# megvii-research/basedet

Hardware: AMD Instinct MI355X
Metric: images/sec training RetinaNet-R50-FPN 1333x800 (higher is better)
Workload: dtype bf16; 1 GPU; retinanet_r50_800x1344 train step (fwd+bwd+allreduce+SGD), DummyLoader boxes, random-init weights, inputs resident in HBM; per_gpu_batch=16, global_batch=16, parallelism=dp1

## Files before the change

basedet_amd/_lib.py:

```python
import ctypes as C
import os

import torch

_HERE = os.path.dirname(os.path.abspath(__file__))
LIB_PATH = os.environ.get("BASEDET_HIP_LIB") or os.path.join(_HERE, "lib", "libbasedet_hip.so")

BD_MAX_SEGS = 8
ABI_VERSION = 105
EPI_RELU, EPI_ADD_BEFORE, EPI_ADD_AFTER, EPI_MASK, EPI_SPARSE = 1, 2, 4, 8, 16


class BasedetHipError(RuntimeError):
    pass


class ConvDesc(C.Structure):
    _fields_ = [
        ("N", C.c_int32), ("Cin", C.c_int32), ("Cout", C.c_int32), ("R", C.c_int32), ("S", C.c_int32),
        ("stride", C.c_int32), ("pad", C.c_int32), ("nseg", C.c_int32),
        ("Hi", C.c_int32 * BD_MAX_SEGS), ("Wi", C.c_int32 * BD_MAX_SEGS),
        ("Ho", C.c_int32 * BD_MAX_SEGS), ("Wo", C.c_int32 * BD_MAX_SEGS),
        ("in_off", C.c_int32 * BD_MAX_SEGS), ("out_off", C.c_int32 * BD_MAX_SEGS),
        ("in_pix_per_img", C.c_int32), ("out_pix_per_img", C.c_int32),
        ("route", C.c_int32 * 4), ("sr_seed", C.c_uint32),
        ("gskip", C.c_int32), ("gskip_ws", C.c_void_p), ("gskip_ws_bytes", C.c_size_t),
        ("gskip_gmap", C.c_void_p), ("gskip_gmap_bytes", C.c_size_t), ("gskip_dxmap", C.c_void_p), ("gskip_dxmap_bytes", C.c_size_t),
        ("gskip_dx_clean", C.c_int32),
    ]


class PackDesc(C.Structure):
    _fields_ = [("w", C.c_void_p), ("row_scale", C.c_void_p), ("w_fwd", C.c_void_p), ("w_dgrad", C.c_void_p),
                ("Cout", C.c_int32), ("RS", C.c_int32), ("Cin", C.c_int32), ("block_start", C.c_int32)]


class ImageDesc(C.Structure):
    _fields_ = [("offset", C.c_int64), ("src_h", C.c_int32), ("src_w", C.c_int32), ("dst_h", C.c_int32), ("dst_w", C.c_int32),
                ("flip", C.c_int32), ("reserved_", C.c_int32 * 1)]


_P, _I, _L, _F, _Z = C.c_void_p, C.c_int, C.c_int64, C.c_float, C.c_size_t
_D = C.POINTER(ConvDesc)

SIGNATURES = {
    "bd_last_error_string": (C.c_char_p, []),
    "bd_version": (_I, []),
    "bd_conv_last_kernel": (C.c_char_p, []),
    "bd_probe_mfma_rate": (_I, [C.c_double, C.POINTER(C.c_double), C.POINTER(C.c_double), _P]),
    "bd_probe_kernel_clock": (_I, [C.c_char_p, _I, C.POINTER(C.c_double), C.POINTER(C.c_double)]),
    "bd_conv2d_fwd": (_I, [_D, _P, _P, _P, _P, _P, _I, _P]),
    "bd_conv2d_dgrad": (_I, [_D, _P, _P, _P, _P, _P, _I, _P]),
    "bd_conv2d_dgrad_gskip_bytes": (_Z, [_D]),
    "bd_conv2d_gskip_map_bytes": (_Z, [_D, _I]),
    "bd_gskip_map_scan": (_I, [_D, _I, _P, _P, _Z, _P]),
    "bd_conv2d_fwd_bits": (_I, [_D, _P, _P, _P, _P, _P, _P, _I, _P]),
    "bd_conv2d_fwd_ex": (_I, [_D, _P, _P, _P, _P, _P, _P, _P, _F, _I, _P]),
    "bd_conv2d_dgrad_ex": (_I, [_D, _P, _P, _P, _P, _P, _P, _P, _F, _I, _P]),
    "bd_conv2d_dgrad_bits": (_I, [_D, _P, _P, _P, _P, _P, _I, _P]),
    "bd_conv2d_wgrad_workspace_bytes": (_Z, [_D]),
    "bd_conv2d_wgrad": (_I, [_D, _P, _P, _P, _P, _I, _P, _Z, _P]),
    "bd_conv2d_wgrad_bias_workspace_bytes": (_Z, [_D]),
    "bd_conv2d_wgrad_bias": (_I, [_D, _P, _P, _P, _P, _P, _I, _P, _Z, _P]),
    "bd_fpn_deconv_pack": (_I, [_P, _I, _P, _P, _P]),
    "bd_fpn_deconv_fwd": (_I, [_P, _P, _P, _P, _I, _I, _I, _I, _I, _I, _P]),
    "bd_fpn_deconv_dgrad": (_I, [_P, _P, _P, _P, _I, _I, _I, _I, _I, _I, _P]),
    "bd_fpn_deconv_wgrad_workspace_bytes": (_Z, [_I, _I, _I, _I]),
    "bd_fpn_deconv_wgrad": (_I, [_P, _P, _P, _I, _P, _Z, _I, _I, _I, _I, _I, _I, _P]),
    "bd_wgrad_queue_create": (_I, [_P]),
    "bd_wgrad_queue_destroy": (_I, [_P]),
    "bd_wgrad_queue_pending": (_I, [_P]),
    "bd_conv2d_wgrad_queued": (_I, [_P, _D, _P, _P, _P, _P, _P, _I, _P, _Z, _P]),
    "bd_wgrad_queue_flush": (_I, [_P, _P]),
    "bd_stem_conv7x7_fwd": (_I, [_I, _I, _I, _P, _P, _P, _P, _P]),
    "bd_stem_pool_fwd": (_I, [_I, _I, _I, _P, _P, _P, _P, _P]),
    "bd_stem_weight_pack": (_I, [_P, _P, _P, _P]),
    "bd_weight_pack": (_I, [_P, _P, _P, _P, _I, _I, _I, _P]),
    "bd_weight_pack_blocks": (_I, [_I, _I, _I]),
    "bd_weight_pack_multi": (_I, [_P, _I, _I, _P]),
    "bd_colsum_workspace_bytes": (_Z, [_I]),
    "bd_colsum_bf16": (_I, [_P, _I, _L, _L, _L, _I, _P, _I, _P, _Z, _P]),
    "bd_pad_normalize": (_I, [_P, _I, _I, _I, _I, _I, _P, _P, _P, _P]),
    "bd_bottleneck_fwd_supported": (_I, [_I, _I, _I, _I, _I, _I, _I]),
    "bd_bottleneck_fwd": (_I, [_I, _I, _I, _I, _I, _I, _P, _P, _P, _P, _P, _P, _P, _P, _P, _P, _P]),
    "bd_h2d_create": (_I, [C.POINTER(C.c_void_p), _I, _I]),
    "bd_h2d_threads": (_I, [_P]),
    "bd_h2d_submit": (_I, [_P, _P, _I, _L, _P, _L, _P]),
    "bd_h2d_destroy": (_I, [_P]),
    "bd_pad_normalize_nchw": (_I, [_P, _I, _I, _I, _I, _I, _P, _P, _P, _P]),
    "bd_resize_pad_normalize": (_I, [_P, _L, C.POINTER(ImageDesc), _I, _I, _I, _P, _P, _P, _P]),
    "bd_maxpool3x3s2_fwd": (_I, [_P, _I, _I, _I, _I, _P, _P]),
    "bd_upsample2x_add_fwd": (_I, [_P, _L, _L, _P, _L, _L, _I, _I, _I, _I, _P]),
    "bd_upsample2x_add_bwd": (_I, [_P, _L, _L, _P, _L, _L, _I, _I, _I, _I, _I, _P]),
    "bd_relu_bf16": (_I, [_P, _P, _L, _P]),
    "bd_relu_bwd_bf16": (_I, [_P, _P, _P, _P, _L, _P]),
    "bd_add_bf16": (_I, [_P, _P, _P, _L, _P]),
    "bd_anchors_generate": (_I, [_I, _I, _I, _F, _P, _I, _P, _P]),
    "bd_points_generate": (_I, [_I, _I, _I, _F, _I, _P, _P]),
    "bd_box_pairwise": (_I, [_P, _I, _P, _I, _I, _P, _P]),
    "bd_box_encode": (_I, [_P, _P, _L, _P, _P, _P, _P]),
    "bd_box_decode": (_I, [_P, _P, _L, _P, _P, _P, _P]),
    "bd_retina_assign_encode": (_I, [_P, _I, _P, _P, _I, _I, _F, _F, _I, _P, _P, _P, _P, _P, _P, _P, _Z, _P]),
    "bd_fcos_assign": (_I, [_P, _I, _P, _P, _P, _I, _F, _P, _P, _I, _I, _P, _P, _P, _P, _P]),
    "bd_ota_assign_workspace_bytes": (_Z, [_I, _I]),
    "bd_ota_assign": (_I, [_P, _I, _P, _P, _I, _P, _I, _P, _P, _P, _I, _I, _F, _F, _F, _F, _I, _P, _P, _P, _P, _P, _Z, _P]),
    "bd_ota_assign_ld": (_I, [_P, _I, _P, _P, _I, _P, _I, _I, _P, _P, _P, _I, _I, _F, _F, _F, _F, _I, _P, _P, _P, _P, _P, _Z, _P]),
    "bd_ota_sinkhorn_workspace_bytes": (_Z, [_I, _I, _I]),
    "bd_ota_assign_sinkhorn": (_I, [_P, _I, _P, _P, _I, _P, _I, _P, _P, _P, _I, _I, _F, _F, _F, _F, _I, _F, _I, _P, _P, _P, _P, _P, _Z, _P]),
    "bd_ota_assign_sinkhorn_ld": (_I, [_P, _I, _P, _P, _I, _P, _I, _I, _P, _P, _P, _I, _I, _F, _F, _F, _F, _I, _F, _I, _P, _P, _P, _P, _P, _Z, _P]),
    "bd_freeanchor_workspace_bytes": (_Z, [_I, _I, _I, _I]),
    "bd_freeanchor_loss_fwd_bwd": (_I, [_P, _P, _I, _I, _P, _I, _I, _P, _P, _I, _I, _P, _P, _F, _I, _F, _F, _F, _F, _P, _P, _P, _P, _Z, _P]),
    "bd_freeanchor_loss_fwd_bwd_ld": (_I, [_P, _I, _P, _I, _I, _P, _I, _I, _P, _P, _I, _I, _P, _P, _F, _I, _F, _F, _F, _F, _P, _P, _P, _P, _Z, _P]),
    "bd_atss_assign_workspace_bytes": (_Z, [_I, _I]),
    "bd_atss_assign": (_I, [_P, _I, _P, _P, _I, _I, _F, _P, _P, _I, _I, _P, _P, _P, _P, _P, _Z, _P]),
    "bd_nms_workspace_bytes": (_Z, [_I]),
    "bd_batched_nms": (_I, [_P, _P, _P, _I, _F, _I, _P, _P, _P, _Z, _P]),
    "bd_focal_loss_fwd_bwd": (_I, [_P, _P, _L, _I, _F, _F, _P, _I, _F, _P, _P, _P]),
    "bd_focal_loss_fwd_bwd_general": (_I, [_P, _P, _L, _I, _F, _F, _P, _I, _F, _P, _P, _P]),
    "bd_focal_loss_fwd_bwd_ld": (_I, [_P, _P, _L, _I, _I, _F, _F, _P, _I, _F, _P, _P, _I, _P]),
    "bd_smooth_l1_fwd_bwd": (_I, [_P, _P, _P, _L, _I, _I, _F, _P, _I, _F, _P, _P, _P]),
    "bd_loss_grid_cap": (_I, []),
    "bd_iou_ltrb_fwd_bwd": (_I, [_P, _P, _P, _P, _L, _I, _P, _F, _P, _P, _P]),
    "bd_giou_ltrb_fwd_bwd": (_I, [_P, _P, _P, _P, _L, _P, _F, _P, _P, _P]),
    "bd_bce_logits_fwd_bwd": (_I, [_P, _I, _I, _P, _P, _L, _P, _P, _P, _P]),
    "bd_groupnorm_workspace_bytes": (_Z, [_I, _I, _I, _L]),
    "bd_groupnorm_fwd": (_I, [_P, _P, _P, _I, _I, _P, _P, _L, _I, _F, _I, _P, _P, _P, _Z, _P]),
    "bd_conv2d_fwd_gnstats_bytes": (_Z, [_D]),
    "bd_conv2d_fwd_gnstats": (_I, [_D, _P, _P, _P, _P, _P, _Z, _P]),
    "bd_groupnorm_fwd_parts": (_I, [_D, _P, _P, _P, _P, _F, _I, _P, _P, _P]),
    "bd_groupnorm_bwd": (_I, [_P, _P, _P, _P, _P, _I, _I, _P, _P, _L, _I, _I, _P, _P, _P, _I, _P, _Z, _P]),
    "bd_fcos_offsets_fwd": (_I, [_P, _I, _P, _I, _I, _P, _P, _P, _L, _P, _P]),
    "bd_fcos_offsets_workspace_bytes": (_Z, []),
    "bd_fcos_offsets_bwd": (_I, [_P, _I, _P, _I, _I, _P, _P, _P, _L, _P, _P, _P, _P, _P, _Z, _P]),
    "bd_rpn_assign_encode": (_I, [_P, _I, _P, _P, _I, _I, _F, _F, _I, _P, _P, _P, _P, _P, _P, _P, _Z, _P]),
    "bd_sample_labels": (_I, [_P, _P, _P, _I, _I, _I, _I, _P, _P]),
    "bd_segment_topk": (_I, [_P, _I, _I, _L, _I, _I, _I, _I, _P, _P, _I, _F, _I, _P, _P, _P, _P]),
    "bd_nms_batched_workspace_bytes": (_Z, [_I, _I]),
    "bd_nms_batched": (_I, [_P, _P, _P, _I, _I, _F, _I, _I, _P, _P, _P, _Z, _P]),
    "bd_rpn_proposals_workspace_bytes": (_Z, [_I, _I, _P, _I, _I, _I]),
    "bd_rpn_proposals": (_I, [_P, _I, _I, _I, _I, _I, _L, _I, _P, _P, _P, _P, _I, _P, _P, _I, _F, _I, _P, _P, _P, _Z, _P]),
    "bd_rpn_proposals_joint": (_I, [_P, _I, _I, _I, _I, _I, _L, _I, _P, _P, _P, _P, _I, _P, _P, _I, _F, _I, _P, _P, _P, _Z, _P]),
    "bd_rcnn_sample_targets": (_I, [_P, _P, _I, _P, _P, _I, _I, _P, _P, _I, _I, _I, _F, _F, _F, _P, _P, _P, _P, _P, _P, _P, _P]),
    "bd_roi_align_fwd": (_I, [_P, _L, _I, _I, _P, _P, _P, _P, _P, _P, _I, _I, _I, _I, _I, _P, _P]),
    "bd_conv1x1_thin_bwd_workspace_bytes": (_Z, []),
    "bd_conv1x1_thin_fwd": (_I, [_P, _P, _P, _L, _I, _I, _P, _P]),
    "bd_conv1x1_thin_bwd": (_I, [_P, _P, _P, _L, _I, _I, _P, _P, _P, _I, _P, _Z, _P]),
    "bd_roi_align_bwd": (_I, [_P, _L, _I, _I, _P, _P, _P, _P, _P, _P, _I, _I, _I, _I, _I, _P, _P]),
    "bd_roi_align_bwd_bf16_workspace_bytes": (_Z, [_I, _I, _P, _P, _I]),
    "bd_roi_align_bwd_bf16": (_I, [_P, _L, _I, _I, _I, _P, _P, _P, _P, _P, _P, _I, _I, _I, _I, _I, _P, _I, _P, _Z, _P]),
    "bd_subsample2x_fwd": (_I, [_P, _L, _L, _I, _I, _P, _L, _L, _I, _I, _P]),
    "bd_subsample2x_bwd_add": (_I, [_P, _L, _L, _P, _L, _L, _I, _I, _I, _I, _P]),
    "bd_f32_to_bf16": (_I, [_P, _P, _L, _P]),
    "bd_f32_to_bf16_add": (_I, [_P, _P, _L, _P]),
    "bd_rpn_loss_fwd_bwd": (_I, [_P, _I, _I, _I, _I, _P, _P, _L, _F, _P, _P, _P, _P]),
    "bd_rcnn_loss_fwd_bwd": (_I, [_P, _I, _I, _I, _P, _P, _I, _F, _P, _P, _P, _P]),
    "bd_det_scores": (_I, [_P, _P, _I, _I, _L, _I, _P, _P]),
    "bd_det_scores_ld": (_I, [_P, _I, _P, _I, _I, _L, _I, _P, _P]),
    "bd_det_select_workspace_bytes": (_Z, [_I, _I, _L, _I, _I]),
    "bd_det_select": (_I, [_P, _P, _I, _I, _I, _L, _I, _I, _P, _P, _I, _F, _P, _P, _P, _P, _Z, _P]),
    "bd_det_select_ld": (_I, [_P, _I, _P, _I, _I, _I, _L, _I, _I, _P, _P, _I, _F, _P, _P, _P, _P, _Z, _P]),
    "bd_rcnn_predict": (_I, [_P, _I, _I, _I, _P, _P, _I, _I, _P, _P, _P, _P, _P]),
    "bd_det_candidates": (_I, [_I, _P, _P, _P, _I, _I, _P, _I, _P, _P, _I, _I, _P, _P, _P, _P, _P, _P, _P]),
    "bd_det_finalize": (_I, [_P, _P, _P, _P, _P, _I, _P, _P, _P, _P, _P]),
    "bd_det_candidates_batched": (_I, [_I, _P, _P, _P, _I, _I, _I, _P, _I, _P, _P, _L, _I, _I, _P, _P, _P, _L, _P, _P, _P, _P]),
    "bd_det_finalize_batched": (_I, [_P, _P, _P, _P, _P, _I, _I, _I, _P, _I, _P, _P, _P, _P]),
    "bd_sgd_momentum_step": (_I, [_P, _P, _P, _L, _F, _F, _F, _F, _P]),
    "bd_ema_update": (_I, [_P, _P, _L, _F, _F, _P]),
    "bd_sgd_momentum_ema_step": (_I, [_P, _P, _P, _P, _L, _F, _F, _F, _F, _F, _F, _P]),
    "bd_swap_f32": (_I, [_P, _P, _L, _P]),
    "bd_clip_grad_value": (_I, [_P, _L, _F, _F, _F, _P]),
    "bd_clip_grad_norm_workspace_bytes": (_Z, []),
    "bd_clip_grad_norm": (_I, [_P, _L, _F, _F, _F, _P, _P, _Z, _P]),
    "bd_quantize_fp8": (_I, [_P, _L, _F, _P, _P]),
    "bd_weight_pack_fp8": (_I, [_P, _P, _I, _I, _I, _F, _P, _P, _P]),
    "bd_conv2d_fwd_fp8": (_I, [_D, _P, _P, _P, _P, _P, _P, _I, _P]),
    "bd_conv2d_fwd_fp8_ex": (_I, [_D, _P, _P, _P, _P, _P, _P, _P, _F, _I, _P]),
    "bd_quantize_bf8": (_I, [_P, _L, _F, _P, C.c_uint32, _P]),
    "bd_absmax_bf16": (_I, [_P, _L, _P, _P]),
    "bd_weight_pack_fp8_t": (_I, [_P, _P, _I, _I, _I, _F, _P, _P, _P]),
    "bd_conv2d_dgrad_fp8": (_I, [_D, _P, _P, _P, _P, _P, _P, _P, _F, _I, _P]),
    "bd_conv2d_wgrad_fp8_workspace_bytes": (_Z, [_D]),
    "bd_conv2d_wgrad_fp8": (_I, [_D, _P, _P, _F, _P, _P, _I, _P, _Z, _P]),
    "bd_conv1x1_fp8": (_I, [_D, _I, _P, _P, _P, _P, _P, _P, _P, _P, _P, _P, _F, _I, _P]),
    "bd_sigmoid_focal_loss_elem": (_I, [_P, _P, _L, _F, _F, _P, _P, _P, _P]),
    "bd_bce_elem": (_I, [_P, _P, _L, _I, _P, _P, _P, _P]),
    "bd_smooth_l1_elem": (_I, [_P, _P, _L, _F, _P, _P, _P, _P]),
    "bd_iou_loss_ltrb": (_I, [_P, _P, _L, _I, _F, _P, _P, _P, _P, _P]),
    "bd_iou_to_loss": (_I, [_P, _L, _I, _F, _P, _P]),
    "bd_matcher_matrix": (_I, [_P, _I, _L, _P, _P, _I, _I, _P, _P, _P, _P]),
    "bd_assign_roi_levels": (_I, [_P, _I, _I, _I, _I, _P, _P]),
    "bd_roi_pool_max_fwd": (_I, [_P, _I, _I, _I, _I, _P, _I, _F, _I, _I, _P, _P]),
    "bd_comm_unique_id": (_I, [_P]),
    "bd_comm_init": (_I, [C.POINTER(C.c_void_p), _P, _I, _I, _I]),
    "bd_comm_rank": (_I, [_P]),
    "bd_comm_world": (_I, [_P]),
    "bd_comm_stream": (_P, [_P]),
    "bd_comm_bcast": (_I, [_P, _P, _Z, _I, _I, _P]),
    "bd_comm_allreduce": (_I, [_P, _P, _Z, _I, _I, _P]),
    "bd_comm_allreduce_async": (_I, [_P, _P, _Z, _I, _I, C.POINTER(C.c_void_p), _I]),
    "bd_comm_allreduce_async_bf16": (_I, [_P, _P, _P, _Z, _I, C.POINTER(C.c_void_p), _I]),
    "bd_comm_wait": (_I, [_P, _P]),
    "bd_comm_destroy": (_I, [_P]),
}

_lib = None


def load():
# ... 51 lines not shown
```

basedet_amd/csrc/conv3x3_pp.hip:

```cpp
#include "conv3x3_pp128_body.h"

namespace {

constexpr int PH = 4, PW = 16, IH = PH + 2, IW = PW + 2;
constexpr int NPATCH = 4;
constexpr int XROWS = NPATCH * IH * IW;
constexpr int X_PITCH = 144;
constexpr int X_BYTES = XROWS * X_PITCH;
constexpr int XPASSES = 7;
constexpr int TILE_CO = 256;
constexpr int W_SLOT = TILE_CO * 128;
constexpr int NSLOT = 3;
constexpr int W_BYTES = NSLOT * W_SLOT;
constexpr int GTAB_TILES = 16;
constexpr int GTAB_BYTES = GTAB_TILES * NPATCH * 32;
constexpr int LDS_BYTES = W_BYTES + X_BYTES + TILE_CO * 4 + GTAB_BYTES;
constexpr int MAX_SEG = BD_MAX_SEGS;
constexpr int TAIL_CO = 64;

struct PSeg { int patch_start, H, W, pw, src_off, dst_off; float inv_pw; };

struct PParams {
    const bf16_raw* src;
    const bf16_raw* w;
    const float* bias;
    const bf16_raw* add;
    const bf16_raw* mask;
    bf16_raw* dst;
    int CK, CO, flags, nseg;
    int src_ppi, dst_ppi;
    unsigned src_bytes;
    int patches_per_img, total_patches, n_tiles;
    int main_grid;
    int px_tiles;
    int tail_end;
    float inv_ppi;
    PSeg seg[MAX_SEG];
    float* gn_part;
    const int* sp_live;
    const int* sp_list;
    const int* sp_count;
    int sp_keep_dead;
    const int* sp_hdr;
    int* sp_ohdr;
    const int* sp_olist;
    int sp_stride, sp_clean;
};

typedef __attribute__((address_space(3))) void lds_void_t;
typedef __attribute__((address_space(1))) const void glb_void_t;

__device__ __forceinline__ int pp_div(int n, int d, float inv) {
    int q = (int)((float)n * inv);
    const int r = n - q * d;
    q += (r >= d) - (r < 0);
    return q;
}

__device__ __forceinline__ int swz(int row, int chunk) { return row * 128 + ((chunk ^ (row & 7)) << 4); }
__device__ __forceinline__ int colperm(int f) { return f < 4 ? 2 * f : (f < 12 ? 2 * (f - 4) + 1 : 2 * (f - 8)); }
__device__ __forceinline__ int xpos(int chunk) { return (chunk >> 2) * 64 + ((((chunk & 1) << 1) | ((chunk >> 1) & 1)) << 4); }

#ifdef BD_PP_STAMP
__device__ unsigned long long g_pp_stamp[64];
__device__ unsigned long long g_pp_span[2048];
#endif
#ifndef BD_PP_ABLATE
#define BD_PP_ABLATE 0
#endif
__device__ unsigned long long g_pp_clk[2];
#define PP_FENCE() __builtin_amdgcn_sched_barrier(0)
#define PP_BARRIER() do { asm volatile("" ::: "memory"); __builtin_amdgcn_s_barrier(); asm volatile("" ::: "memory"); } while (0)

template <int MODE, bool GNS = false, bool SPARSE = false>
__global__ __launch_bounds__(512, 1) void conv3x3_pp_kernel(const PParams p) {
    extern __shared__ __attribute__((aligned(16))) unsigned char smem[];
    if (!SPARSE && (int)blockIdx.x >= p.main_grid) {
        pp128::body<MODE, TAIL_CO>(p, smem, (int)blockIdx.x - p.main_grid, (int)gridDim.x - p.main_grid, p.total_patches, p.tail_end,
                                   (p.CO + TAIL_CO - 1) / TAIL_CO);
        return;
    }
    if (!SPARSE && blockIdx.x == 0 && threadIdx.x == 0) bd_clk_mark(g_pp_clk, false);
    unsigned char* wbuf = smem;
    unsigned char* xbuf = smem + W_BYTES;
    float* sbias = reinterpret_cast<float*>(smem + W_BYTES + X_BYTES);

#ifdef BD_PP_STAMP
    int st_n = 0;
    const bool st_on = blockIdx.x == 100 % gridDim.x && threadIdx.x == 0;
#define PP_STAMP() do { if (st_on && st_n < 62) g_pp_stamp[st_n] = __builtin_amdgcn_s_memtime(); ++st_n; } while (0)
    PP_STAMP();
    if (st_on) g_pp_stamp[62] = __builtin_amdgcn_s_memrealtime();
    if (threadIdx.x == 0 && blockIdx.x < 1024) g_pp_span[2 * blockIdx.x] = __builtin_amdgcn_s_memrealtime();
#else
#define PP_STAMP() do { } while (0)
#endif
    const int tid = threadIdx.x, lane = tid & 63, wave = __builtin_amdgcn_readfirstlane(tid >> 6);
    const int wm = wave >> 2, wp = wave & 3;
    int bid = blockIdx.x;
    {
        const int nwg = p.main_grid;
        const int q = nwg >> 3, r = nwg & 7, xcd = bid & 7;
        bid = (xcd < r ? xcd * (q + 1) : r * (q + 1) + (xcd - r) * q) + (bid >> 3);
    }
    const int ct = bid % p.n_tiles;
    int pt = bid / p.n_tiles;
    const int pt_step = p.main_grid / p.n_tiles;
    const int co0 = ct * TILE_CO;

    auto zero_dead = [&](int z0, int zn) {
        if (p.sp_keep_dead) return;
        const int cpp = p.CO >> 3;
        const int items = PH * PW * cpp;
        int zt = p.total_patches;
        const int* plist = nullptr;
        if (p.sp_clean) {
            const int oc = __builtin_amdgcn_readfirstlane(p.sp_ohdr[0]) & 1;
            const int pc = __builtin_amdgcn_readfirstlane(p.sp_ohdr[2 + oc]);
            zt = pc < 0 ? 0 : (pc < zt ? pc : zt);
            plist = p.sp_olist + oc * p.sp_stride;
        }
        for (int k0 = 0; z0 + k0 * zn < zt; k0 += 512) {
            const int k = k0 + wave * 64 + lane;
            const int idx = z0 + k * zn;
            int q = idx;
            if (plist) q = idx < zt ? plist[idx] : -1;
            const bool dead = idx < zt && q >= 0 && q < p.total_patches && p.sp_live[q] == 0;
            unsigned long long m = __ballot(dead);
            while (m) {
                const int l = __builtin_ctzll(m);
                m &= m - 1;
                const int qq = __builtin_amdgcn_readfirstlane(__shfl(q, l, 64));
                const int n = qq / p.patches_per_img, rem = qq - n * p.patches_per_img;
                int sgi = 0;
#pragma unroll
                for (int z = 1; z < MAX_SEG; ++z)
                    if (z < p.nseg && rem >= p.seg[z].patch_start) sgi = z;
                const int H = p.seg[sgi].H, W = p.seg[sgi].W, pwn = p.seg[sgi].pw;
                const int local = rem - p.seg[sgi].patch_start, by = local / pwn, bx = local - by * pwn;
                const long long img = (long long)n * p.dst_ppi + p.seg[sgi].dst_off;
                for (int i = lane; i < items; i += 64) {
                    const int px = i / cpp, ch = i - px * cpp;
                    const int y = by * PH + px / PW, x = bx * PW + (px & (PW - 1));
                    if (y < H && x < W)
                        *reinterpret_cast<u32x4_t*>(p.dst + (img + (long long)y * W + x) * p.CO + ch * 8) = (u32x4_t){0u, 0u, 0u, 0u};
                }
            }
        }
    };
    int n_px = p.px_tiles, n_live = p.total_patches;
    int z_first = 0;
    const int* sp_list = p.sp_list;
    if constexpr (SPARSE) {
        if (p.sp_ohdr && blockIdx.x == 0 && threadIdx.x == 0) p.sp_ohdr[1] = 0;
        const int cur = p.sp_hdr ? __builtin_amdgcn_readfirstlane(p.sp_hdr[0]) & 1 : 0;
        const int* cntp = p.sp_hdr ? p.sp_hdr + 2 + cur : p.sp_count;
        n_live = __builtin_amdgcn_readfirstlane(*cntp);
        sp_list += cur * p.sp_stride;
        n_live = __builtin_amdgcn_readfirstlane(n_live < 0 ? 0 : (n_live < p.total_patches ? n_live : p.total_patches));
        n_px = (n_live + NPATCH - 1) / NPATCH;
        z_first = n_px * p.n_tiles < p.main_grid ? n_px * p.n_tiles : p.main_grid;
        if (pt >= n_px) {
            zero_dead(bid - z_first, p.main_grid - z_first);
            return;
        }
    }

    constexpr unsigned X_NONE = 0x80000000u;
    const int x_lds0 = (tid >> 3) * X_PITCH + xpos(tid & 7);
    unsigned x_off[XPASSES];

    int* gtab = reinterpret_cast<int*>(smem + W_BYTES + X_BYTES + TILE_CO * 4);
    const int pt_first = pt;
    auto build_table = [&](int k0) {
        const int k = k0 + (lane >> 2);
        const int ptile = pt_first + k * pt_step;
        int pid = ptile * NPATCH + (lane & (NPATCH - 1));
        if (SPARSE) pid = (ptile < n_px && pid < n_live) ? sp_list[pid] : p.total_patches;
        int vH = 0, vW = 0, vy = 0, vx = 0, vs = 0, vd = 0;
        if (ptile < n_px && pid < p.total_patches) {
            const int n = pp_div(pid, p.patches_per_img, p.inv_ppi);
            const int rem = pid - n * p.patches_per_img;
            int g_start = p.seg[0].patch_start, g_H = p.seg[0].H, g_W = p.seg[0].W, g_pw = p.seg[0].pw;
            int g_src = p.seg[0].src_off, g_dst = p.seg[0].dst_off;
            float g_inv = p.seg[0].inv_pw;
#pragma unroll
            for (int q = 1; q < MAX_SEG; ++q) {
                const bool in = q < p.nseg && rem >= p.seg[q].patch_start;
                g_start = in ? p.seg[q].patch_start : g_start; g_H = in ? p.seg[q].H : g_H; g_W = in ? p.seg[q].W : g_W;
                g_pw = in ? p.seg[q].pw : g_pw; g_src = in ? p.seg[q].src_off : g_src; g_dst = in ? p.seg[q].dst_off : g_dst;
                g_inv = in ? p.seg[q].inv_pw : g_inv;
            }
            const int local = rem - g_start;
            const int by = pp_div(local, g_pw, g_inv), bx = local - by * g_pw;
            vy = by * PH; vx = bx * PW; vH = g_H; vW = g_W;
            vs = n * p.src_ppi + g_src;
            vd = n * p.dst_ppi + g_dst;
        }
        typedef __attribute__((ext_vector_type(4))) int i32x4_t;
        i32x4_t* e = reinterpret_cast<i32x4_t*>(gtab + ((k & (GTAB_TILES - 1)) * NPATCH + (lane & (NPATCH - 1))) * 8);
        e[0] = (i32x4_t){vy, vx, vH, vW};
        e[1] = (i32x4_t){vs, vd, 0, 0};
    };
    auto decode = [&](int k, int& e_oy0, int& e_px0, int& e_H, int& e_W, int& e_dst) {
        int py0[NPATCH], px0[NPATCH], pH[NPATCH], pWd[NPATCH];
        int psrc[NPATCH], pdst[NPATCH];
        int tq = tid;
        asm volatile("" : "+v"(tq));
        {
            typedef __attribute__((ext_vector_type(4))) int i32x4_t;
            const i32x4_t* e = reinterpret_cast<const i32x4_t*>(gtab + ((k & (GTAB_TILES - 1)) * NPATCH + (tq & (NPATCH - 1))) * 8);
            const i32x4_t e0 = e[0], e1 = e[1];
#pragma unroll
            for (int q = 0; q < NPATCH; ++q) {
                py0[q] = __builtin_amdgcn_readlane(e0[0], q); px0[q] = __builtin_amdgcn_readlane(e0[1], q);
                pH[q] = __builtin_amdgcn_readlane(e0[2], q); pWd[q] = __builtin_amdgcn_readlane(e0[3], q);
                psrc[q] = __builtin_amdgcn_readlane(e1[0], q); pdst[q] = __builtin_amdgcn_readlane(e1[1], q);
            }
        }
#pragma unroll
        for (int k = 0; k < XPASSES; ++k) {
            const int row = (tq >> 3) + 64 * k;
            unsigned off = X_NONE;
            if (row < XROWS) {
                const int lo = (64 * k) / (IH * IW), hi = (64 * k + 63) / (IH * IW) < NPATCH ? (64 * k + 63) / (IH * IW) : NPATCH - 1;
                const bool up = row >= hi * (IH * IW);
                const int pk = up ? hi : lo;
                const int rr = row - pk * (IH * IW);
                const int iy = rr / IW, ix = rr - iy * IW;
                const int qy = up ? py0[hi] : py0[lo], qx = up ? px0[hi] : px0[lo], H = up ? pH[hi] : pH[lo];
                const int W = up ? pWd[hi] : pWd[lo], qs = up ? psrc[hi] : psrc[lo];
                const int y = qy - 1 + iy, x = qx - 1 + ix;
                if (y >= 0 && x >= 0 && y < H && x < W) off = (unsigned)((qs + y * W + x) * p.CK + (tq & 7) * 8) * 2u;
            }
            x_off[k] = off;
        }
        e_oy0 = py0[0]; e_px0 = px0[0]; e_H = pH[0]; e_W = pWd[0]; e_dst = pdst[0];
#pragma unroll
        for (int q = 1; q < NPATCH; ++q)
            if (wp == q) { e_oy0 = py0[q]; e_px0 = px0[q]; e_H = pH[q]; e_W = pWd[q]; e_dst = pdst[q]; }
    };
    int c_oy0, c_px0, c_H, c_W, c_dst;
    int kt = 0;
    if (wave == 0) build_table(0);
    asm volatile("s_waitcnt lgkmcnt(0)" ::: "memory");
    PP_BARRIER();
    decode(0, c_oy0, c_px0, c_H, c_W, c_dst);
    const __amdgpu_buffer_rsrc_t x_rsrc =
        __builtin_amdgcn_make_buffer_rsrc(const_cast<bf16_raw*>(p.src), 0, p.src_bytes, 0x00020000);
    u32x4_t rx[XPASSES];
    auto load_x = [&](int cb) {
        int so = cb * 128;
        asm volatile("" : "+s"(so));
        const bool dead = cb * 64 + (tid & 7) * 8 >= p.CK;
#pragma unroll
        for (int k = 0; k < XPASSES; ++k) rx[k] = __builtin_amdgcn_raw_buffer_load_b128(x_rsrc, dead ? X_NONE : x_off[k], so, 0);
    };
    auto write_x = [&]() {
#pragma unroll
        for (int k = 0; k < XPASSES; ++k)
            if (k < XPASSES - 1 || (tid >> 3) + 64 * k < XROWS)
                *reinterpret_cast<u32x4_t*>(xbuf + x_lds0 + k * (64 * X_PITCH)) = rx[k];
    };

    unsigned dma_src[4];
#pragma unroll
    for (int k = 0; k < 4; ++k) {
        const int pc = wave + 8 * k;
        const int lrow = 8 * pc + (lane >> 3);
        const int chunk = (lane & 7) ^ (lane >> 3);
        const int rho = lrow & 15;
        int co = co0 + (lrow & 192) + 32 * ((lrow >> 5) & 1) + 8 * (rho >> 2) + 4 * ((lrow >> 4) & 1) + (rho & 3);
        if (co >= p.CO) co = p.CO - 1;
        dma_src[k] = (unsigned)(co * 9 * p.CK + chunk * 8) * 2u;
    }
    const __amdgpu_buffer_rsrc_t w_rsrc =
        __builtin_amdgcn_make_buffer_rsrc(const_cast<bf16_raw*>(p.w), 0, (unsigned)(p.CO * 9 * p.CK) * 2u, 0x00020000);
    bool dma_on = true;
    auto dma_piece = [&](int tap, int cb, int slot, int k) {
        if ((BD_PP_ABLATE & 2) && !dma_on) return;
        unsigned char* l = wbuf + slot * W_SLOT + (wave + 8 * k) * 1024;
        int so = (tap * p.CK + cb * 64) * 2;
        asm volatile("" : "+s"(so));
        __builtin_amdgcn_raw_ptr_buffer_load_lds(w_rsrc, (lds_void_t*)l, 16, dma_src[k], so, 0, 0);
    };

    f32x4_t acc[8][4];

    const int frow = lane & 15, fchunk = lane >> 4;
    const unsigned char* a_base[2];
#pragma unroll
    for (int kk = 0; kk < 2; ++kk) a_base[kk] = wbuf + swz(wm * 128 + frow, kk * 4 + fchunk);
    typedef __attribute__((address_space(3))) const unsigned char lds_u8_t;
    typedef __attribute__((address_space(3))) const bf16x8_t lds_bf16x8_t;
    unsigned a_hi[2];
#pragma unroll
    for (int kk = 0; kk < 2; ++kk) {
        a_hi[kk] = (unsigned)(size_t)(lds_u8_t*)(a_base[kk]) + 2 * W_SLOT;
        asm volatile("" : "+v"(a_hi[kk]));
    }
    const unsigned char* b_base = xbuf + (wp * (IH * IW) + colperm(frow)) * X_PITCH + xpos(fchunk);

    bf16x8_t fa[8], fb[4];
    auto load_a = [&](int kk, int slot) {
#pragma unroll
        for (int i = 0; i < 8; ++i) {
            if (slot == 2) fa[i] = *(lds_bf16x8_t*)(size_t)(a_hi[kk] + i * 2048);
// ... 271 lines not shown
                if (add_before) {
#pragma unroll
                    for (int k = 0; k < 4; ++k) { v[2 * k] += bf_lo(a4[k]); v[2 * k + 1] += bf_hi(a4[k]); }
                }
                if (do_relu) {
#pragma unroll
                    for (int k = 0; k < 8; ++k) v[k] = fmaxf(v[k], 0.f);
                }
                if (do_mask) {
#pragma unroll
                    for (int k = 0; k < 4; ++k) {
                        if (!(bf_lo(m4[k]) > 0.f)) v[2 * k] = 0.f;
                        if (!(bf_hi(m4[k]) > 0.f)) v[2 * k + 1] = 0.f;
                    }
                }
                if (add_after) {
#pragma unroll
                    for (int k = 0; k < 4; ++k) { v[2 * k] += bf_lo(a4[k]); v[2 * k + 1] += bf_hi(a4[k]); }
                }
                u32x4_t o;
#pragma unroll
                for (int k = 0; k < 4; ++k) o[k] = pack_bf2(v[2 * k], v[2 * k + 1]);
                *reinterpret_cast<u32x4_t*>(p.dst + idx) = o;
            }
        }
    }
    }
    PP_STAMP();
    if (!more) break;
    ++kt;
    pt = pt_next;
    c_oy0 = n_oy0; c_px0 = n_px0; c_H = n_H; c_W = n_W; c_dst = n_dst;
    PP_FENCE();
    PP_STAMP();
    }
    if constexpr (SPARSE) {
        if (z_first == p.main_grid) zero_dead(bid, p.main_grid);
    }
    if (!SPARSE && blockIdx.x == 0 && threadIdx.x == 0) bd_clk_mark(g_pp_clk, true);
#ifdef BD_PP_STAMP
    if (st_on) { g_pp_stamp[63] = __builtin_amdgcn_s_memrealtime(); g_pp_stamp[61] = __builtin_amdgcn_s_memtime(); }
    if (threadIdx.x == 0 && blockIdx.x < 1024) { asm volatile("s_waitcnt vmcnt(0)" ::: "memory"); g_pp_span[2 * blockIdx.x + 1] = __builtin_amdgcn_s_memrealtime(); }
#endif
}

}

BD_KNOB int g_pp_tail_split = 1;
BD_KNOB int g_pp_persistent = 1;
extern BD_KNOB int g_patch_pp;
int bd_gskip_patches(const bd_conv_desc* d, int ph, int pw);
void bd_gskip_fill(const bd_conv_desc* d, int side, const void* t, const int* live_in, int* map, hipStream_t stream);
void bd_gskip_scan(const bd_conv_desc* d, const void* g, int ph, int pw, int* mask, hipStream_t stream);
void bd_gskip_compact(const bd_conv_desc* d, int ph, int pw, const int* mask, int* live, int* list, int* count, hipStream_t stream);

extern "C" size_t bd_conv2d_dgrad_gskip_bytes(const bd_conv_desc* d) {
    if (!d || d->nseg < 1 || d->nseg > BD_MAX_SEGS || !(d->R == 3 && d->S == 3 && d->stride == 1 && d->pad == 1)) return 0;
    return ((size_t)3 * bd_gskip_patches(d, PH, PW) + 4) * sizeof(int);
}

static bool pp_sparse_epilogue(int flags, const void* add, const void* dst) {
    const bool in_place = (flags & BD_EPI_ADD_BEFORE) && add && add == dst;
    return !(flags & BD_EPI_ADD_AFTER) && (!((flags & BD_EPI_ADD_BEFORE) && add) || (in_place && !(flags & BD_EPI_MASK)));
}

bool bd_conv3x3_pp_maps_ok(const bd_conv_desc* d, int flags, const void* add, const void* dst) {
    if (g_patch_pp < 2 || !(d->R == 3 && d->S == 3 && d->stride == 1 && d->pad == 1)) return false;
    if (d->Cout % 8 != 0 || d->Cin <= 128 || d->Cin % 8 != 0) return false;
    if ((long long)d->N * d->out_pix_per_img * d->Cout * 2 >= 0x7fffffffll || (long long)d->N * d->in_pix_per_img >= 0x7fffffffll ||
        (long long)d->Cin * 9 * d->Cout >= 0x7fffffffll) return false;
    for (int s = 0; s < d->nseg; ++s)
        if (d->Hi[s] != d->Ho[s] || d->Wi[s] != d->Wo[s]) return false;
    if (bd_gskip_patches(d, PH, PW) >= (1 << 24)) return false;
    const bool in_place = (flags & BD_EPI_ADD_BEFORE) && add && add == dst;
    if (d->gskip_dxmap && in_place) return false;
    return pp_sparse_epilogue(flags, add, dst);
}

static int pp_launch(const bd_conv_desc* d, int mode, const void* src, const void* w, const float* bias, const void* add,
                     const void* mask, void* dst, int flags, float* gn_part, hipStream_t stream) {
    PParams p{};
    p.gn_part = gn_part;
    p.CK = mode == 0 ? d->Cin : d->Cout;
    p.CO = mode == 0 ? d->Cout : d->Cin;
    p.src_ppi = mode == 0 ? d->in_pix_per_img : d->out_pix_per_img;
    p.dst_ppi = mode == 0 ? d->out_pix_per_img : d->in_pix_per_img;
    if (p.CK % 8 != 0 || p.CO <= 128 || p.CO % 8 != 0) return 1;
    if ((long long)d->N * p.src_ppi * p.CK * 2 >= 0x7fffffffll || (long long)d->N * p.dst_ppi >= 0x7fffffffll ||
        (long long)p.CO * 9 * p.CK >= 0x7fffffffll) return 1;
    p.src = (const bf16_raw*)src; p.w = (const bf16_raw*)w; p.bias = bias;
    p.add = (const bf16_raw*)add; p.mask = (const bf16_raw*)mask; p.dst = (bf16_raw*)dst;
    p.flags = flags; p.nseg = d->nseg;
    p.src_bytes = (unsigned)((long long)d->N * p.src_ppi * p.CK * 2);
    int ps = 0;
    for (int s = 0; s < d->nseg; ++s) {
        PSeg& sg = p.seg[s];
        sg.patch_start = ps; sg.H = d->Ho[s]; sg.W = d->Wo[s]; sg.pw = cdiv(d->Wo[s], PW); sg.inv_pw = 1.0f / (float)sg.pw;
        sg.src_off = mode == 0 ? d->in_off[s] : d->out_off[s];
        sg.dst_off = mode == 0 ? d->out_off[s] : d->in_off[s];
        ps += cdiv(d->Ho[s], PH) * sg.pw;
    }
    p.patches_per_img = ps;
    p.inv_ppi = 1.0f / (float)ps;
    p.total_patches = ps * d->N;
    if (p.total_patches >= (1 << 24)) return 1;
    p.n_tiles = cdiv(p.CO, TILE_CO);
    int grid = cdiv(p.total_patches, NPATCH) * p.n_tiles;
    int tail_wgs = 0;
    int px_tiles = cdiv(p.total_patches, NPATCH);
    p.tail_end = p.total_patches;
    const int num_cus = bd_num_cus();
    const bool in_place = (flags & BD_EPI_ADD_BEFORE) && add && add == dst;
    const bool sparse = mode == 1 && d->gskip && !gn_part && pp_sparse_epilogue(flags, add, dst);
    if (g_pp_tail_split && !sparse && !gn_part && p.n_tiles == 1 && px_tiles > num_cus) {
        const int r = px_tiles % num_cus;
        if (r > 0 && r * (TILE_CO / TAIL_CO) <= num_cus) {
            px_tiles -= r;
            p.total_patches = px_tiles * NPATCH;
            tail_wgs = cdiv(p.tail_end - p.total_patches, NPATCH) * cdiv(p.CO, TAIL_CO);
        }
    }
    p.px_tiles = px_tiles;
    p.main_grid = px_tiles * p.n_tiles;
    if (g_pp_persistent) {
        const int g1 = (num_cus / p.n_tiles) * p.n_tiles;
        const int rounds = cdiv(px_tiles * p.n_tiles, g1 * GTAB_TILES);
        if (g1 * rounds < p.main_grid) p.main_grid = g1 * rounds;
    }
    {
        const int grid128 = cdiv(p.total_patches, NPATCH) * cdiv(p.CO, 128);
        if (!gn_part && g_patch_pp < 2 && 3 * cdiv(grid, 256) >= 2 * cdiv(grid128, 256)) return 1;
    }
    BD_ONCE_PER_DEVICE(
        (void)hipFuncSetAttribute(reinterpret_cast<const void*>(&conv3x3_pp_kernel<0>), hipFuncAttributeMaxDynamicSharedMemorySize, LDS_BYTES);
        (void)hipFuncSetAttribute(reinterpret_cast<const void*>(&conv3x3_pp_kernel<1>), hipFuncAttributeMaxDynamicSharedMemorySize, LDS_BYTES);
        (void)hipFuncSetAttribute(reinterpret_cast<const void*>(&conv3x3_pp_kernel<1, false, true>), hipFuncAttributeMaxDynamicSharedMemorySize,
                                  LDS_BYTES));
    bd_note_kernel("conv3x3_pp_kernel");
    if (sparse) {
        const int tot = p.total_patches;
        p.sp_keep_dead = in_place ? 1 : 0;
        p.sp_stride = tot;
        if (d->gskip_gmap) {
            BdGskipMap gm;
            bd_gskip_map_layout(d, 0, &gm);
            const int* m = (const int*)d->gskip_gmap;
            p.sp_hdr = m; p.sp_live = m + gm.live; p.sp_list = m + gm.list;
        } else {
            int* mk = (int*)d->gskip_ws;
            p.sp_live = mk + tot; p.sp_list = mk + 2 * tot; p.sp_count = mk + 3 * tot;
            bd_gskip_scan(d, src, PH, PW, mk, stream);
            bd_gskip_compact(d, PH, PW, mk, mk + tot, mk + 2 * tot, mk + 3 * tot, stream);
        }
        if (d->gskip_dxmap) {
            BdGskipMap xm;
            bd_gskip_map_layout(d, 1, &xm);
            p.sp_ohdr = (int*)d->gskip_dxmap; p.sp_olist = p.sp_ohdr + xm.list;
            p.sp_clean = d->gskip_dx_clean ? 1 : 0;
        }
        hipLaunchKernelGGL((conv3x3_pp_kernel<1, false, true>), dim3(p.main_grid), dim3(512), LDS_BYTES, stream, p);
        if (d->gskip_dxmap) bd_gskip_fill(d, 1, dst, p.sp_live, (int*)d->gskip_dxmap, stream);
    } else if (gn_part) {
        BD_ONCE_PER_DEVICE((void)hipFuncSetAttribute(reinterpret_cast<const void*>(&conv3x3_pp_kernel<0, true>), hipFuncAttributeMaxDynamicSharedMemorySize, LDS_BYTES));
        hipLaunchKernelGGL((conv3x3_pp_kernel<0, true>), dim3(p.main_grid), dim3(512), LDS_BYTES, stream, p);
    } else if (mode == 0) hipLaunchKernelGGL((conv3x3_pp_kernel<0>), dim3(p.main_grid + tail_wgs), dim3(512), LDS_BYTES, stream, p);
    else hipLaunchKernelGGL((conv3x3_pp_kernel<1>), dim3(p.main_grid + tail_wgs), dim3(512), LDS_BYTES, stream, p);
    return 0;
}

int bd_pp_clk_read(unsigned long long* out2, int reset) {
    if (hipMemcpyFromSymbol(out2, HIP_SYMBOL(g_pp_clk), 16) != hipSuccess) return 1;
    if (reset) { const unsigned long long z[2] = {0, 0}; if (hipMemcpyToSymbol(HIP_SYMBOL(g_pp_clk), z, 16) != hipSuccess) return 1; }
    return 0;
}

#ifdef BD_PP_STAMP
extern "C" int bd_debug_pp_stamp(unsigned long long* out2) {
    return hipMemcpyFromSymbol(out2, HIP_SYMBOL(g_pp_stamp), 512) == hipSuccess ? 0 : 1;
}
extern "C" int bd_debug_pp_span(unsigned long long* out2048) {
    return hipMemcpyFromSymbol(out2048, HIP_SYMBOL(g_pp_span), 2048 * 8) == hipSuccess ? 0 : 1;
}
#endif

int bd_conv3x3_pp_launch(const bd_conv_desc* d, int mode, const void* src, const void* w, const float* bias, const void* add,
                         const void* mask, void* dst, int flags, hipStream_t stream) {
    return pp_launch(d, mode, src, w, bias, add, mask, dst, flags, nullptr, stream);
}

int bd_conv3x3_pp_patch_starts(const bd_conv_desc* d, int* starts) {
    int ps = 0;
    for (int s = 0; s < d->nseg; ++s) { starts[s] = ps; ps += cdiv(d->Ho[s], PH) * cdiv(d->Wo[s], PW); }
    starts[d->nseg] = ps;
    return ps;
}

extern "C" size_t bd_conv2d_fwd_gnstats_bytes(const bd_conv_desc* d) {
    if (!d || d->nseg < 1 || d->nseg > BD_MAX_SEGS) return 0;
    int starts[BD_MAX_SEGS + 1];
    return (size_t)d->N * bd_conv3x3_pp_patch_starts(d, starts) * 32 * 2 * sizeof(float);
}

extern "C" int bd_conv2d_fwd_gnstats(const bd_conv_desc* d, const void* x, const void* w_packed, const float* bias, void* y, float* part,
                                     size_t part_bytes, bd_stream_t stream) {
    BD_ROUTE(d);
    BD_REQUIRE(d && x && w_packed && y && part, "conv2d_fwd_gnstats: null pointer");
    BD_REQUIRE(d->R == 3 && d->S == 3 && d->stride == 1 && d->pad == 1 && d->Cout == 256 && d->Cin % 64 == 0,
               "conv2d_fwd_gnstats: 3x3 / stride 1 / pad 1 into 256 channels (GroupNorm(32, 256)) only; got %dx%d s%d p%d %d -> %d", d->R, d->S,
               d->stride, d->pad, d->Cin, d->Cout);
    for (int s = 0; s < d->nseg; ++s)
        BD_REQUIRE(d->Hi[s] == d->Ho[s] && d->Wi[s] == d->Wo[s], "conv2d_fwd_gnstats: level %d changes size", s);
    if (part_bytes < bd_conv2d_fwd_gnstats_bytes(d)) { bd_set_error("conv2d_fwd_gnstats: statistics buffer too small"); return BD_EWORKSPACE; }
    if (pp_launch(d, 0, x, w_packed, bias, nullptr, nullptr, y, 0, part, (hipStream_t)stream) != 0) {
        bd_set_error("conv2d_fwd_gnstats: shape not taken by conv3x3_pp_kernel (tensor too large for 32-bit offsets?)");
        return BD_EINVAL;
    }
    BD_CHECK_LAUNCH("bd_conv2d_fwd_gnstats");
    return BD_OK;
}
```

basedet_amd/csrc/conv_igemm.hip:

```cpp
#include "igemm_params.h"

using namespace igemm;

namespace {

template <int BK>
struct Cfg {
    static constexpr int CHUNKS = BK / 8;
    static constexpr int ROWS_PER_PASS = 256 / CHUNKS;
    static constexpr int PASSES = 128 / ROWS_PER_PASS;
    static constexpr int LDS_STRIDE = BK == 64 ? 160 : 64;
    static constexpr int TILE_BYTES = 128 * LDS_STRIDE;
    __device__ static __forceinline__ int off(int row, int chunk) {
        if constexpr (BK == 64) return row * LDS_STRIDE + chunk * 16;
        else return row * 64 + ((chunk ^ ((row >> 1) & 3)) << 4);
    }
};

template <int BK, bool PRE, bool BUF>
__global__ __launch_bounds__(256) void conv_igemm_kernel(const IgemmParams p) {
    using C = Cfg<BK>;
    extern __shared__ __attribute__((aligned(16))) unsigned char smem[];
    unsigned char* tiles = smem;
    unsigned int* s_tapmask = reinterpret_cast<unsigned int*>(smem);
// ... 386 lines not shown
bool bd_conv3x3_pp_maps_ok(const bd_conv_desc* d, int flags, const void* add, const void* dst);

extern BD_KNOB int g_patch_dma;
extern BD_KNOB int g_patch_pp;
extern BD_KNOB int g_patch_pp128;
extern BD_KNOB int g_conv1x1_s2;
extern BD_KNOB int g_pp_tail_split;
extern BD_KNOB int g_pp_persistent;
static int bd_route_patch3x3(int enable) {
#ifdef BD_AB_SKIP
    g_skip_s2_3x3 = (enable >> 4) & 1;
#else
    if ((enable >> 4) & 1) {
        bd_set_error("bd_conv_desc.route[1]: bit 4 (skip the 3x3 / stride-2 launches: a timing A/B that leaves stale outputs) exists in "
                     "-DBD_AB_SKIP diagnostic builds only");
        return BD_EINVAL;
    }
#endif
    g_use_patch3x3 = enable & 1; g_bk32_for_1x1 = (enable >> 1) & 1;
    g_patch_dma = ((enable >> 3) & 1) ^ 1;
    g_patch_pp = ((enable >> 6) & 1) ? 0 : (((enable >> 7) & 1) ? 1 : 2);
    g_patch_pp128 = ((enable >> 9) & 1) ? -1 : ((enable >> 8) & 1);
    g_bk32_s2 = ((enable >> 10) & 1) ^ 1;
    g_igemm_prefetch_epi = ((enable >> 5) & 1) ^ 1;
    g_igemm_buf = ((enable >> 11) & 1) ^ 1;
    g_conv1x1_s2 = ((enable >> 12) & 1) ^ 1;
    g_pp_tail_split = ((enable >> 13) & 1) ^ 1;
    g_pp_persistent = ((enable >> 14) & 1) ^ 1;
    if ((enable >> 16) & 1) {
        bd_set_error("bd_conv_desc.route[1]: bit 16 (conv_igemm_wide.hip) is gone since round 6");
        return BD_EINVAL;
    }
    return BD_OK;
}

int bd_route_dense1x1(int depth);
int bd_route_wgrad(int use_tr);
extern BD_KNOB int g_fp8_patch;

BdRouteScope::BdRouteScope(const bd_conv_desc* d) : rc(BD_OK) {
    const int r0 = d ? d->route[0] : 0, r1 = d ? d->route[1] : 0, r2 = d ? d->route[2] : 0, r3 = d ? d->route[3] : 0;
    if (r0 < 0 || r1 < 0 || r2 < 0 || r3 < 0) {
        bd_set_error("bd_conv_desc.route: negative word (0 = the library's choice, otherwise the route + 1)");
        rc = BD_EINVAL;
        return;
    }
    if ((rc = bd_route_dense1x1(r0 ? r0 - 1 : 1)) != BD_OK) return;
    if ((rc = bd_route_patch3x3(r1 ? r1 - 1 : 3)) != BD_OK) return;
    if ((rc = bd_route_wgrad(r2 ? r2 - 1 : 1)) != BD_OK) return;
    g_fp8_patch = r3 ? (r3 - 1 != 0) : 1;
    g_fp8_sr_seed = d ? d->sr_seed : 0u;
}

int bd_conv1x1_dense_launch(const void* x, const void* w, const float* bias, const void* add, const void* mask, const unsigned* maskbits,
                            void* y, unsigned* ybits, void* y8, float q_scale, int y8_bf8, long long M, int CK, int CO, int flags,
                            hipStream_t stream);

int bd_conv1x1_s2_launch(const bd_conv_desc* d, int mode, const void* src, const void* w, const float* bias, const void* add, const void* mask,
                         const unsigned* maskbits, void* dst, int flags, hipStream_t stream);
namespace {
bool is_dense_1x1(const bd_conv_desc* d) {
    return d->R == 1 && d->S == 1 && d->stride == 1 && d->pad == 0 && d->nseg == 1 && d->in_off[0] == 0 && d->out_off[0] == 0 &&
           d->in_pix_per_img == d->Hi[0] * d->Wi[0] && d->out_pix_per_img == d->Ho[0] * d->Wo[0];
}
}

static int conv2d_fwd_impl(const bd_conv_desc* d, const void* x, const void* w_packed, const float* bias, const void* add, void* y,
                           unsigned* ybits, void* y8, float q_scale, int flags, bd_stream_t stream) {
    if (int e = check_desc(d)) return e;
    BD_REQUIRE(x && w_packed && y, "conv2d_fwd: null pointer");
    BD_REQUIRE(d->Cin % 8 == 0, "conv2d_fwd: Cin=%d must be a multiple of 8", d->Cin);
    BD_REQUIRE(d->Cout % 8 == 0, "conv2d_fwd: Cout=%d must be a multiple of 8", d->Cout);
    BD_REQUIRE(!(flags & BD_EPI_MASK), "conv2d_fwd: BD_EPI_MASK is a dgrad-only flag");
    if (is_dense_1x1(d) &&
        bd_conv1x1_dense_launch(x, w_packed, bias, add, nullptr, nullptr, y, ybits, y8, q_scale, 0, (long long)d->N * d->out_pix_per_img,
                                d->Cin, d->Cout, flags, (hipStream_t)stream) == 0) {
        BD_CHECK_LAUNCH("bd_conv2d_fwd(dense 1x1)");
        return BD_OK;
    }
    if (!ybits && !y8 && d->stride == 2 && d->R == 1 &&
        bd_conv1x1_s2_launch(d, 0, x, w_packed, bias, add, nullptr, nullptr, y, flags, (hipStream_t)stream) == 0) {
        BD_CHECK_LAUNCH("bd_conv2d_fwd(1x1 stride 2)");
        return BD_OK;
    }
    BD_REQUIRE(ybits == nullptr && y8 == nullptr, "conv2d_fwd_bits / _ex: the bit-packed ReLU mask and the e4m3 twin are written by the dense "
               "1x1 kernel only (1x1 / stride 1 over one dense level, Cout %% 32 == 0, tensors < 2 GB)");
#ifdef BD_AB_SKIP
    if (g_skip_s2_3x3 && d->R == 3 && d->S == 3 && d->stride == 2) return BD_OK;
#endif
    if (g_use_patch3x3 && is_3x3s1(d)) {
        bd_conv3x3_patch_launch(d, 0, x, w_packed, bias, add, nullptr, y, flags, (hipStream_t)stream);
        BD_CHECK_LAUNCH("bd_conv2d_fwd(3x3 patch)");
        return BD_OK;
    }
    IgemmParams p{};
    p.src = (const bf16_raw*)x; p.w = (const bf16_raw*)w_packed; p.bias = bias;
    p.add = (const bf16_raw*)add; p.mask = nullptr; p.dst = (bf16_raw*)y;
    p.CK = d->Cin; p.CO = d->Cout; p.R = d->R; p.S = d->S; p.stride = d->stride; p.pad = d->pad;
    p.mode = 0; p.flags = flags;
    p.nsub = d->nseg;
    long long m = 0;
    for (int s = 0; s < d->nseg; ++s) {
        SubSeg& ss = p.sub[s];
        ss.m_start = (int)m;
        ss.Hs = d->Ho[s]; ss.Ws = d->Wo[s]; ss.y0 = 0; ss.x0 = 0; ss.step = 1;
        ss.Wd = d->Wo[s]; ss.dst_off = d->out_off[s];
        ss.Hsrc = d->Hi[s]; ss.Wsrc = d->Wi[s]; ss.src_off = d->in_off[s];
        ss.inv_per_img = 1.0f / (float)(ss.Hs * ss.Ws); ss.inv_ws = 1.0f / (float)ss.Ws;
        m += (long long)d->N * d->Ho[s] * d->Wo[s];
    }
    BD_REQUIRE(m < (1ll << 24), "conv2d_fwd: too many pixels (2^24 limit of the fast index decode)");
    p.linear_dst = (d->nseg == 1 && d->out_off[0] == 0 && d->out_pix_per_img == d->Ho[0] * d->Wo[0]) ? 1 : 0;
    p.linear_src = (p.linear_dst && d->R == 1 && d->S == 1 && d->stride == 1 && d->pad == 0 && d->in_off[0] == 0 &&
                    d->in_pix_per_img == d->Hi[0] * d->Wi[0]) ? 1 : 0;
    p.M = (int)m;
    p.src_pix_per_img = d->in_pix_per_img; p.dst_pix_per_img = d->out_pix_per_img;
    set_buffer_sizes(p, d->N);
    p.m_tiles = cdiv(p.M, TILE_P); p.n_tiles = cdiv(p.CO, TILE_C);
    if (p.CK > 32 && !(g_bk32_for_1x1 && p.R * p.S == 1) && !(g_bk32_s2 && p.stride == 2 && p.m_tiles * p.n_tiles >= 512))
        launch_igemm<64>(p, (hipStream_t)stream);
    else launch_igemm<32>(p, (hipStream_t)stream);
    BD_CHECK_LAUNCH("bd_conv2d_fwd");
    return BD_OK;
}

extern "C" int bd_conv2d_fwd(const bd_conv_desc* d, const void* x, const void* w_packed, const float* bias,
                             const void* add, void* y, int flags, bd_stream_t stream) {
    BD_ROUTE(d);
    return conv2d_fwd_impl(d, x, w_packed, bias, add, y, nullptr, nullptr, 1.f, flags, stream);
}

extern "C" int bd_conv2d_fwd_ex(const bd_conv_desc* d, const void* x, const void* w_packed, const float* bias, const void* add, void* y,
                                uint32_t* ybits, void* y8, float q_scale, int flags, bd_stream_t stream) {
    BD_ROUTE(d);
    return conv2d_fwd_impl(d, x, w_packed, bias, add, y, ybits, y8, q_scale, flags, stream);
}

extern "C" int bd_conv2d_fwd_bits(const bd_conv_desc* d, const void* x, const void* w_packed, const float* bias, const void* add, void* y,
                                  uint32_t* ybits, int flags, bd_stream_t stream) {
    BD_ROUTE(d);
    BD_REQUIRE(ybits != nullptr, "conv2d_fwd_bits: null ybits");
    return conv2d_fwd_impl(d, x, w_packed, bias, add, y, ybits, nullptr, 1.f, flags, stream);
}

static int conv2d_dgrad_impl(const bd_conv_desc* d, const void* g, const void* w_packed_t, const void* add, const void* mask,
                             const unsigned* maskbits, void* dx, void* dx8, float q_scale, int flags, bd_stream_t stream) {
    if (int e = check_desc(d)) return e;
    BD_REQUIRE(g && w_packed_t && dx, "conv2d_dgrad: null pointer");
    if (d->gskip && is_3x3s1(d) && !d->gskip_gmap) {
        const size_t need = bd_conv2d_dgrad_gskip_bytes(d);
        BD_REQUIRE(d->gskip_ws && d->gskip_ws_bytes >= need, "conv2d_dgrad: gskip scratch %zu < required %zu bytes (or NULL)",
                   (size_t)d->gskip_ws_bytes, need);
    }
    if (d->gskip_gmap || d->gskip_dxmap || d->gskip_dx_clean) {
        BD_REQUIRE(d->gskip && is_3x3s1(d) && g_use_patch3x3 && !maskbits && !dx8 && bd_conv3x3_pp_maps_ok(d, flags, add, dx),
                   "conv2d_dgrad: liveness maps need gskip on a 3x3 / stride 1 / pad 1 descriptor into more than 128 channels with an overwriting "
                   "(or, without gskip_dxmap, in-place accumulating) epilogue on the default route");
        BD_REQUIRE(!d->gskip_gmap || d->gskip_gmap_bytes >= bd_conv2d_gskip_map_bytes(d, 0), "conv2d_dgrad: gskip_gmap %zu < required %zu bytes",
                   (size_t)d->gskip_gmap_bytes, bd_conv2d_gskip_map_bytes(d, 0));
        BD_REQUIRE(!d->gskip_dxmap || d->gskip_dxmap_bytes >= bd_conv2d_gskip_map_bytes(d, 1), "conv2d_dgrad: gskip_dxmap %zu < required %zu bytes",
                   (size_t)d->gskip_dxmap_bytes, bd_conv2d_gskip_map_bytes(d, 1));
        BD_REQUIRE(!d->gskip_dx_clean || d->gskip_dxmap, "conv2d_dgrad: gskip_dx_clean needs gskip_dxmap (the list the promise refers to)");
    }
    if (d->stride == 1) flags &= ~BD_EPI_SPARSE;
    BD_REQUIRE(d->Cout % 8 == 0, "conv2d_dgrad: Cout=%d must be a multiple of 8 (pad the gradient)", d->Cout);
    BD_REQUIRE(d->Cin % 8 == 0, "conv2d_dgrad: Cin=%d must be a multiple of 8", d->Cin);
    BD_REQUIRE(!(flags & BD_EPI_RELU), "conv2d_dgrad: BD_EPI_RELU is a forward-only flag");
    if (is_dense_1x1(d) &&
        bd_conv1x1_dense_launch(g, w_packed_t, nullptr, add, mask, maskbits, dx, nullptr, dx8, q_scale, 1, (long long)d->N * d->in_pix_per_img,
                                d->Cout, d->Cin, flags, (hipStream_t)stream) == 0) {
        BD_CHECK_LAUNCH("bd_conv2d_dgrad(dense 1x1)");
        return BD_OK;
    }
    if (!dx8 && d->stride == 2 && d->R == 1 &&
        bd_conv1x1_s2_launch(d, 1, g, w_packed_t, nullptr, add, mask, maskbits, dx, flags, (hipStream_t)stream) == 0) {
        BD_CHECK_LAUNCH("bd_conv2d_dgrad(1x1 stride 2)");
        return BD_OK;
    }
    BD_REQUIRE(maskbits == nullptr && dx8 == nullptr, "conv2d_dgrad_bits / _ex: the bit-packed ReLU mask is read, and the e5m2 twin written, by "
               "the dense 1x1 kernel only (1x1 / stride 1 over one dense level, Cin %% 32 == 0, tensors < 2 GB)");
#ifdef BD_AB_SKIP
    if (g_skip_s2_3x3 && d->R == 3 && d->S == 3 && d->stride == 2) return BD_OK;
#endif
    if (g_use_patch3x3 && is_3x3s1(d)) {
        bd_conv3x3_patch_launch(d, 1, g, w_packed_t, nullptr, add, mask, dx, flags, (hipStream_t)stream);
        BD_CHECK_LAUNCH("bd_conv2d_dgrad(3x3 patch)");
        return BD_OK;
    }
    IgemmParams p{};
    p.src = (const bf16_raw*)g; p.w = (const bf16_raw*)w_packed_t; p.bias = nullptr;
    p.add = (const bf16_raw*)add; p.mask = (const bf16_raw*)mask; p.dst = (bf16_raw*)dx;
    p.CK = d->Cout; p.CO = d->Cin; p.R = d->R; p.S = d->S; p.stride = d->stride; p.pad = d->pad;
    p.mode = 1; p.flags = flags;
    long long m = 0;
    int ns = 0;
    const int st = d->stride;
    const bool sparse = (flags & BD_EPI_SPARSE) && st > 1;
    BD_REQUIRE(!(flags & BD_EPI_SPARSE) || ((flags & BD_EPI_ADD_BEFORE) && add == dx),
               "conv2d_dgrad: BD_EPI_SPARSE needs an in-place accumulate (BD_EPI_ADD_BEFORE with add == dx)");
    p.flags = flags & ~BD_EPI_SPARSE;
    for (int s = 0; s < d->nseg; ++s) {
        for (int qy = 0; qy < st; ++qy)
            for (int qx = 0; qx < st; ++qx) {
                const int Hs = (d->Hi[s] - qy + st - 1) / st, Ws = (d->Wi[s] - qx + st - 1) / st;
                if (Hs <= 0 || Ws <= 0) continue;
                if (sparse) {
                    bool ry = false, rx = false;
                    for (int r = 0; r < d->R; ++r) ry = ry || ((qy + d->pad - r) % st + st) % st == 0;
                    for (int c = 0; c < d->S; ++c) rx = rx || ((qx + d->pad - c) % st + st) % st == 0;
                    if (!(ry && rx)) continue;
                }
                BD_REQUIRE(ns < MAX_SUB, "conv2d_dgrad: too many sub-segments (levels x stride^2 > %d)", MAX_SUB);
                SubSeg& ss = p.sub[ns++];
                ss.m_start = (int)m;
                ss.Hs = Hs; ss.Ws = Ws; ss.y0 = qy; ss.x0 = qx; ss.step = st;
                ss.Wd = d->Wi[s]; ss.dst_off = d->in_off[s];
                ss.Hsrc = d->Ho[s]; ss.Wsrc = d->Wo[s]; ss.src_off = d->out_off[s];
                ss.inv_per_img = 1.0f / (float)(Hs * Ws); ss.inv_ws = 1.0f / (float)Ws;
                m += (long long)d->N * Hs * Ws;
            }
    }
    p.nsub = ns;
    BD_REQUIRE(m < (1ll << 24), "conv2d_dgrad: too many pixels (2^24 limit of the fast index decode)");
    p.linear_dst = (d->nseg == 1 && st == 1 && d->in_off[0] == 0 && d->in_pix_per_img == d->Hi[0] * d->Wi[0]) ? 1 : 0;
    p.linear_src = (p.linear_dst && d->R == 1 && d->S == 1 && d->pad == 0 && d->out_off[0] == 0 &&
                    d->out_pix_per_img == d->Ho[0] * d->Wo[0]) ? 1 : 0;
    p.M = (int)m;
    p.src_pix_per_img = d->out_pix_per_img; p.dst_pix_per_img = d->in_pix_per_img;
    set_buffer_sizes(p, d->N);
    p.m_tiles = cdiv(p.M, TILE_P); p.n_tiles = cdiv(p.CO, TILE_C);
    if (p.CK > 32 && !(g_bk32_for_1x1 && p.R * p.S == 1) && !(g_bk32_s2 && p.stride == 2 && p.m_tiles * p.n_tiles >= 512))
        launch_igemm<64>(p, (hipStream_t)stream);
    else launch_igemm<32>(p, (hipStream_t)stream);
    BD_CHECK_LAUNCH("bd_conv2d_dgrad");
    return BD_OK;
}

extern "C" int bd_conv2d_dgrad(const bd_conv_desc* d, const void* g, const void* w_packed_t, const void* add,
                               const void* mask, void* dx, int flags, bd_stream_t stream) {
    BD_ROUTE(d);
    return conv2d_dgrad_impl(d, g, w_packed_t, add, mask, nullptr, dx, nullptr, 1.f, flags, stream);
}

extern "C" int bd_conv2d_dgrad_ex(const bd_conv_desc* d, const void* g, const void* w_packed_t, const void* add, const void* mask,
                                  const uint32_t* maskbits, void* dx, void* dx8, float q_scale, int flags, bd_stream_t stream) {
    BD_ROUTE(d);
    return conv2d_dgrad_impl(d, g, w_packed_t, add, maskbits ? nullptr : mask, maskbits, dx, dx8, q_scale,
                             maskbits ? (flags | BD_EPI_MASK) : flags, stream);
}

extern "C" int bd_conv2d_dgrad_bits(const bd_conv_desc* d, const void* g, const void* w_packed_t, const void* add, const uint32_t* maskbits,
                                    void* dx, int flags, bd_stream_t stream) {
    BD_ROUTE(d);
    BD_REQUIRE(maskbits != nullptr, "conv2d_dgrad_bits: null maskbits");
    return conv2d_dgrad_impl(d, g, w_packed_t, add, nullptr, maskbits, dx, nullptr, 1.f, flags | BD_EPI_MASK, stream);
}
```

basedet_amd/csrc/gskip.hip:

```cpp
#include "common.h"

namespace {

enum { GS_ANY = 1, GS_TOP = 2, GS_BOT = 4, GS_LEFT = 8, GS_RIGHT = 16, GS_TL = 32, GS_TR = 64, GS_BL = 128, GS_BR = 256 };

struct GsSeg { int patch_start, H, W, pw, off; };

struct GsParams {
    const bf16_raw* g;
    int* mask;
    int C, ppi, ph, pw_px, nseg, patches_per_img, total;
    GsSeg seg[BD_MAX_SEGS];
};

__device__ __forceinline__ int gs_level(const GsParams& p, int rem) {
    int s = 0;
#pragma unroll
    for (int k = 1; k < BD_MAX_SEGS; ++k)
        if (k < p.nseg && rem >= p.seg[k].patch_start) s = k;
    return s;
}

__global__ __launch_bounds__(256) void gskip_scan_kernel(const GsParams p) {
    __shared__ int sbits;
    const int tid = threadIdx.x;
    const int pid = blockIdx.x;
    const int n = pid / p.patches_per_img, rem = pid - n * p.patches_per_img;
    const int s = gs_level(p, rem);
    const int H = p.seg[s].H, W = p.seg[s].W, pwn = p.seg[s].pw;
    const int local = rem - p.seg[s].patch_start, by = local / pwn, bx = local - by * pwn;
    const int y0 = by * p.ph, x0 = bx * p.pw_px;
    const int cpp = p.C >> 3;
    const int items = p.ph * p.pw_px * cpp;
    const long long img = (long long)n * p.ppi + p.seg[s].off;
    if (tid == 0) sbits = 0;
    __syncthreads();
    int bits = 0;
    constexpr int U = 8;
    for (int b = 0; b < items; b += 256 * U) {
        u32x4_t v[U];
        int pix[U];
#pragma unroll
        for (int k = 0; k < U; ++k) {
            const int i = b + k * 256 + tid;
            v[k] = (u32x4_t){0u, 0u, 0u, 0u};
            pix[k] = -1;
            if (i < items) {
                const int px = i / cpp, ch = i - px * cpp;
                const int py = px / p.pw_px, pxx = px - py * p.pw_px;
                const int y = y0 + py, x = x0 + pxx;
                if (y < H && x < W) {
                    v[k] = *reinterpret_cast<const u32x4_t*>(p.g + (img + (long long)y * W + x) * p.C + ch * 8);
                    pix[k] = px;
                }
            }
        }
#pragma unroll
        for (int k = 0; k < U; ++k) {
            if (pix[k] >= 0 && (v[k][0] | v[k][1] | v[k][2] | v[k][3])) {
                const int py = pix[k] / p.pw_px, pxx = pix[k] - py * p.pw_px;
                const bool t = py == 0, bo = py == p.ph - 1, l = pxx == 0, r = pxx == p.pw_px - 1;
                bits |= GS_ANY | (t ? GS_TOP : 0) | (bo ? GS_BOT : 0) | (l ? GS_LEFT : 0) | (r ? GS_RIGHT : 0) | (t && l ? GS_TL : 0) |
                        (t && r ? GS_TR : 0) | (bo && l ? GS_BL : 0) | (bo && r ? GS_BR : 0);
            }
        }
    }
#pragma unroll
    for (int m = 32; m >= 1; m >>= 1) bits |= __shfl_xor(bits, m, 64);
    if ((tid & 63) == 0 && bits) atomicOr(&sbits, bits);
    __syncthreads();
    if (tid == 0) p.mask[pid] = sbits;
}

template <bool FRESH>
__device__ __forceinline__ int gs_mask(const int* m, int i) {
    if (FRESH) return __hip_atomic_load(m + i, __ATOMIC_RELAXED, __HIP_MEMORY_SCOPE_AGENT);
    return m[i];
}

template <bool FRESH>
__device__ __forceinline__ void gs_compact_body(const GsParams& p, int* live, int* list, int* count, int* wsum) {
    constexpr int KP = 8;
    const int tid = threadIdx.x, wv = tid >> 6, ln = tid & 63;
    int base = 0;
    for (int c0 = 0; c0 < p.total; c0 += 1024 * KP) {
        int lv[KP];
#pragma unroll
        for (int j = 0; j < KP; ++j) {
            const int q = c0 + tid * KP + j;
            lv[j] = 0;
            if (q < p.total) {
                const int n = q / p.patches_per_img, rem = q - n * p.patches_per_img;
                const int s = gs_level(p, rem);
                const int pwn = p.seg[s].pw, rows = (p.seg[s].H + p.ph - 1) / p.ph;
                const int local = rem - p.seg[s].patch_start, by = local / pwn, bx = local - by * pwn;
                const int* m = p.mask + (long long)n * p.patches_per_img + p.seg[s].patch_start;
                const bool up = by > 0, dn = by + 1 < rows, lf = bx > 0, rt = bx + 1 < pwn;
                int v = gs_mask<FRESH>(m, by * pwn + bx) & GS_ANY;
                if (up) v |= gs_mask<FRESH>(m, (by - 1) * pwn + bx) & GS_BOT;
                if (dn) v |= gs_mask<FRESH>(m, (by + 1) * pwn + bx) & GS_TOP;
                if (lf) v |= gs_mask<FRESH>(m, by * pwn + bx - 1) & GS_RIGHT;
                if (rt) v |= gs_mask<FRESH>(m, by * pwn + bx + 1) & GS_LEFT;
                if (up && lf) v |= gs_mask<FRESH>(m, (by - 1) * pwn + bx - 1) & GS_BR;
                if (up && rt) v |= gs_mask<FRESH>(m, (by - 1) * pwn + bx + 1) & GS_BL;
                if (dn && lf) v |= gs_mask<FRESH>(m, (by + 1) * pwn + bx - 1) & GS_TR;
                if (dn && rt) v |= gs_mask<FRESH>(m, (by + 1) * pwn + bx + 1) & GS_TL;
                lv[j] = v != 0;
            }
        }
        int cnt = 0;
#pragma unroll
        for (int j = 0; j < KP; ++j) cnt += lv[j];
        int inc = cnt;
#pragma unroll
        for (int o = 1; o < 64; o <<= 1) {
            const int y = __shfl_up(inc, o, 64);
            if (ln >= o) inc += y;
        }
        if (ln == 63) wsum[wv] = inc;
        __syncthreads();
        int off = base + inc - cnt, tot = 0;
#pragma unroll
        for (int w = 0; w < 16; ++w) {
            off += w < wv ? wsum[w] : 0;
            tot += wsum[w];
        }
#pragma unroll
        for (int j = 0; j < KP; ++j) {
            const int q = c0 + tid * KP + j;
            if (q < p.total) live[q] = lv[j];
            if (lv[j]) list[off++] = q;
        }
        base += tot;
        __syncthreads();
    }
    if (tid == 0) *count = base;
}

__global__ __launch_bounds__(1024) void gskip_compact_kernel(const GsParams p, int* live, int* list, int* count) {
    __shared__ int wsum[16];
    gs_compact_body<false>(p, live, list, count, wsum);
}

enum { GM_HDR = 8 };

struct GmSeg { int H, W, off, s4, s8, ss; };

struct GmParams {
    const bf16_raw* t;
    const int* live_in;
    int* map;
    int C, ppi, nseg, pi4, pi8, pis, tot4, tot8;
    GmSeg seg[BD_MAX_SEGS];
};

__global__ __launch_bounds__(1024) void gskip_fill_kernel(const GmParams p, const GsParams cp, int total) {
    __shared__ int sbits, slast;
    __shared__ int wsum[16];
    const int tid = threadIdx.x;
    int* m4 = p.map + GM_HDR;
    int* m8 = m4 + p.tot4;
    const int cpp = p.C >> 3;
    const int items = 4 * 16 * cpp;
    for (int pid = blockIdx.x; pid < total; pid += gridDim.x) {
        const int n = pid / p.pis, rem = pid - n * p.pis;
        int s = 0;
#pragma unroll
        for (int k = 1; k < BD_MAX_SEGS; ++k)
            if (k < p.nseg && rem >= p.seg[k].ss) s = k;
        const int H = p.seg[s].H, W = p.seg[s].W;
        const int sc = (W + 15) >> 4, r4 = (H + 3) >> 2, c8 = (W + 7) >> 3;
        const int local = rem - p.seg[s].ss, sy = local / sc, sx = local - sy * sc;
        int q4[2], q8[2];
        bool ok4[2], ok8[2], lv[2];
#pragma unroll
        for (int h = 0; h < 2; ++h) {
            ok4[h] = 2 * sy + h < r4;
            q4[h] = n * p.pi4 + p.seg[s].s4 + (2 * sy + h) * sc + sx;
            ok8[h] = 2 * sx + h < c8;
            q8[h] = n * p.pi8 + p.seg[s].s8 + sy * c8 + 2 * sx + h;
            lv[h] = ok4[h] && (p.live_in == nullptr || p.live_in[q4[h]] != 0);
        }
        int b = 0;
        if (lv[0] || lv[1]) {
            if (tid == 0) sbits = 0;
            __syncthreads();
            const long long img = (long long)n * p.ppi + p.seg[s].off;
            int bits = 0;
#pragma unroll
            for (int h = 0; h < 2; ++h) {
                if (!lv[h]) continue;
                for (int i = tid; i < items; i += 1024) {
                    const int px = i / cpp, ch = i - px * cpp;
                    const int py = px >> 4, pxx = px & 15;
                    const int y = 8 * sy + 4 * h + py, x = 16 * sx + pxx;
                    if (y < H && x < W) {
                        const u32x4_t v = *reinterpret_cast<const u32x4_t*>(p.t + (img + (long long)y * W + x) * p.C + ch * 8);
                        if (v[0] | v[1] | v[2] | v[3]) {
                            const bool t = py == 0, bo = py == 3, l = pxx == 0, r = pxx == 15;
                            const int w = GS_ANY | (t ? GS_TOP : 0) | (bo ? GS_BOT : 0) | (l ? GS_LEFT : 0) | (r ? GS_RIGHT : 0) |
                                          (t && l ? GS_TL : 0) | (t && r ? GS_TR : 0) | (bo && l ? GS_BL : 0) | (bo && r ? GS_BR : 0);
                            bits |= (w << (9 * h)) | (1 << (18 + (pxx >> 3)));
                        }
                    }
                }
            }
#pragma unroll
            for (int m = 32; m >= 1; m >>= 1) bits |= __shfl_xor(bits, m, 64);
            if ((tid & 63) == 0 && bits) atomicOr(&sbits, bits);
            __syncthreads();
            b = sbits;
            __syncthreads();
        }
        if (tid == 0) {
            if (ok4[0]) m4[q4[0]] = b & 511;
            if (ok4[1]) m4[q4[1]] = (b >> 9) & 511;
            if (ok8[0]) m8[q8[0]] = (b >> 18) & 1;
            if (ok8[1]) m8[q8[1]] = (b >> 19) & 1;
        }
    }
    if (tid == 0) {
        __builtin_amdgcn_fence(__ATOMIC_RELEASE, "agent");
        slast = atomicAdd(p.map + 1, 1) == (int)gridDim.x - 1;
    }
    __syncthreads();
    if (!slast) return;
    __builtin_amdgcn_fence(__ATOMIC_ACQUIRE, "agent");
    const int nxt = (p.map[0] & 1) ^ 1;
    int* live = m8 + p.tot8;
    gs_compact_body<true>(cp, live, live + p.tot4 * (1 + nxt), p.map + 2 + nxt, wsum);
    if (tid == 0) { p.map[0] = nxt; p.map[1] = 0; }
}

GsParams gs_params(const bd_conv_desc* d, int ph, int pw, int side = 0) {
    GsParams p{};
    p.C = side ? d->Cin : d->Cout; p.ppi = side ? d->in_pix_per_img : d->out_pix_per_img; p.ph = ph; p.pw_px = pw; p.nseg = d->nseg;
    int ps = 0;
    for (int s = 0; s < d->nseg; ++s) {
        GsSeg& sg = p.seg[s];
        const int H = side ? d->Hi[s] : d->Ho[s], W = side ? d->Wi[s] : d->Wo[s];
        sg.patch_start = ps; sg.H = H; sg.W = W; sg.pw = cdiv(W, pw); sg.off = side ? d->in_off[s] : d->out_off[s];
        ps += cdiv(H, ph) * sg.pw;
    }
    p.patches_per_img = ps;
    p.total = ps * d->N;
    return p;
}

}

int bd_gskip_patches(const bd_conv_desc* d, int ph, int pw) {
    return gs_params(d, ph, pw).total;
}

void bd_gskip_scan(const bd_conv_desc* d, const void* g, int ph, int pw, int* mask, hipStream_t stream) {
    GsParams p = gs_params(d, ph, pw);
    p.g = (const bf16_raw*)g; p.mask = mask;
    if (p.total > 0) hipLaunchKernelGGL(gskip_scan_kernel, dim3(p.total), dim3(256), 0, stream, p);
}

void bd_gskip_compact(const bd_conv_desc* d, int ph, int pw, const int* mask, int* live, int* list, int* count, hipStream_t stream) {
    GsParams p = gs_params(d, ph, pw);
    p.mask = const_cast<int*>(mask);
    hipLaunchKernelGGL(gskip_compact_kernel, dim3(1), dim3(1024), 0, stream, p, live, list, count);
}

void bd_gskip_map_layout(const bd_conv_desc* d, int side, BdGskipMap* out) {
    const int p4 = gs_params(d, 4, 16, side).total, p8 = gs_params(d, 8, 8, side).total;
    out->p4 = p4; out->p8 = p8;
    out->m4 = GM_HDR; out->m8 = GM_HDR + p4; out->live = out->m8 + p8; out->list = out->live + p4;
    out->ints = (size_t)GM_HDR + (size_t)4 * p4 + p8;
}

extern "C" size_t bd_conv2d_gskip_map_bytes(const bd_conv_desc* d, int of_dx) {
    if (!d || d->nseg < 1 || d->nseg > BD_MAX_SEGS || !(d->R == 3 && d->S == 3 && d->stride == 1 && d->pad == 1)) return 0;
    BdGskipMap m;
    bd_gskip_map_layout(d, of_dx ? 1 : 0, &m);
    return m.ints * sizeof(int);
}

void bd_gskip_fill(const bd_conv_desc* d, int side, const void* t, const int* live_in, int* map, hipStream_t stream) {
    const GsParams g4 = gs_params(d, 4, 16, side), g8 = gs_params(d, 8, 8, side), gs = gs_params(d, 8, 16, side);
    GmParams p{};
    p.t = (const bf16_raw*)t; p.live_in = live_in; p.map = map;
    p.C = g4.C; p.ppi = g4.ppi; p.nseg = g4.nseg;
    p.pi4 = g4.patches_per_img; p.pi8 = g8.patches_per_img; p.pis = gs.patches_per_img; p.tot4 = g4.total; p.tot8 = g8.total;
    for (int s = 0; s < g4.nseg; ++s)
        p.seg[s] = GmSeg{g4.seg[s].H, g4.seg[s].W, g4.seg[s].off, g4.seg[s].patch_start, g8.seg[s].patch_start, gs.seg[s].patch_start};
    GsParams cp = g4;
    cp.mask = map + GM_HDR;
    const int grid = gs.total < 128 ? gs.total : 128;
    if (grid > 0) hipLaunchKernelGGL(gskip_fill_kernel, dim3(grid), dim3(1024), 0, stream, p, cp, gs.total);
}

extern "C" int bd_gskip_map_scan(const bd_conv_desc* d, int of_dx, const void* t, void* map, size_t map_bytes, bd_stream_t stream) {
    BD_REQUIRE(d && t && map, "gskip_map_scan: null pointer");
    const size_t need = bd_conv2d_gskip_map_bytes(d, of_dx);
    BD_REQUIRE(need > 0, "gskip_map_scan: liveness maps belong to 3x3 / stride 1 / pad 1 descriptors");
    BD_REQUIRE(map_bytes >= need, "gskip_map_scan: map %zu < required %zu bytes", map_bytes, need);
    const int side = of_dx ? 1 : 0;
    BdGskipMap m;
    bd_gskip_map_layout(d, side, &m);
    int* mp = (int*)map;
    if (hipMemsetAsync(mp, 0, GM_HDR * sizeof(int), (hipStream_t)stream) != hipSuccess) { bd_set_error("gskip_map_scan: memset failed"); return BD_ELAUNCH; }
    GsParams p4 = gs_params(d, 4, 16, side), p8 = gs_params(d, 8, 8, side);
    p4.g = p8.g = (const bf16_raw*)t;
    p4.mask = mp + m.m4; p8.mask = mp + m.m8;
    if (p4.total > 0) {
        hipLaunchKernelGGL(gskip_scan_kernel, dim3(p4.total), dim3(256), 0, (hipStream_t)stream, p4);
        hipLaunchKernelGGL(gskip_scan_kernel, dim3(p8.total), dim3(256), 0, (hipStream_t)stream, p8);
    }
    hipLaunchKernelGGL(gskip_compact_kernel, dim3(1), dim3(1024), 0, (hipStream_t)stream, p4, mp + m.live, mp + m.list, mp + 2);
    BD_CHECK_LAUNCH("bd_gskip_map_scan");
    return BD_OK;
}
```

basedet_amd/csrc/image_ops.hip:

```cpp
#include <stdarg.h>

#include <cmath>
#include "common.h"

static thread_local std::string g_bd_error = "";
int bd_num_cus() {
    static std::mutex mu;
    static int cached[256] = {0};
    int dev = 0;
    if (hipGetDevice(&dev) != hipSuccess || dev < 0 || dev > 255) return 256;
    std::lock_guard<std::mutex> g(mu);
    if (!cached[dev]) {
        int n = 0;
        cached[dev] = (hipDeviceGetAttribute(&n, hipDeviceAttributeMultiprocessorCount, dev) == hipSuccess && n > 0) ? n : 256;
    }
    return cached[dev];
}

void bd_set_error(const char* fmt, ...) {
    char buf[512];
    va_list ap;
    va_start(ap, fmt);
    vsnprintf(buf, sizeof(buf), fmt, ap);
    va_end(ap);
    g_bd_error = buf;
}
extern "C" const char* bd_last_error_string(void) { return g_bd_error.c_str(); }
static thread_local const char* g_bd_last_kernel = "";
void bd_note_kernel(const char* name) { g_bd_last_kernel = name; }
extern "C" const char* bd_conv_last_kernel(void) { return g_bd_last_kernel; }
extern "C" int bd_version(void) { return 105; }

namespace {

constexpr int HALO_Y = 3, HALO_X = 4;

__global__ void pad_normalize_kernel(const float* __restrict__ in, int N, int H, int W, int Hp, int Wp,
                                     float m0, float m1, float m2, float s0, float s1, float s2,
                                     bf16_raw* __restrict__ out) {
    const int Hb = Hp + 2 * HALO_Y, Wb = Wp + 2 * HALO_X;
    const long long total = (long long)N * Hb * Wb;
    for (long long i = (long long)blockIdx.x * blockDim.x + threadIdx.x; i < total; i += (long long)gridDim.x * blockDim.x) {
        const int xb = (int)(i % Wb);
        const long long t = i / Wb;
        const int yb = (int)(t % Hb);
        const int n = (int)(t / Hb);
        const int y = yb - HALO_Y, x = xb - HALO_X;
        u32x2_t o = {0u, 0u};
        if (y >= 0 && y < Hp && x >= 0 && x < Wp) {
            float v0 = 0.f, v1 = 0.f, v2 = 0.f;
            if (y < H && x < W) {
                const long long base = ((long long)n * 3 * H + y) * W + x;
                v0 = in[base]; v1 = in[base + (long long)H * W]; v2 = in[base + 2ll * H * W];
            }
            o[0] = pack_bf2((v0 - m0) / s0, (v1 - m1) / s1);
            o[1] = pack_bf2((v2 - m2) / s2, 0.f);
        }
        *reinterpret_cast<u32x2_t*>(out + i * 4) = o;
    }
}

__global__ void pad_normalize_nchw_kernel(const float* __restrict__ in, int N, int H, int W, int Hp, int Wp,
                                          float m0, float m1, float m2, float s0, float s1, float s2,
                                          float* __restrict__ out) {
    const long long total = (long long)N * 3 * Hp * Wp;
    for (long long i = (long long)blockIdx.x * blockDim.x + threadIdx.x; i < total; i += (long long)gridDim.x * blockDim.x) {
        const int x = (int)(i % Wp);
        long long t = i / Wp;
        const int y = (int)(t % Hp);
        t /= Hp;
        const int c = (int)(t % 3);
        const int n = (int)(t / 3);
        float v = 0.f;
        if (y < H && x < W) v = in[(((long long)n * 3 + c) * H + y) * W + x];
        const float m = c == 0 ? m0 : (c == 1 ? m1 : m2);
        const float s = c == 0 ? s0 : (c == 1 ? s1 : s2);
        out[i] = (v - m) / s;
    }
}

__device__ __forceinline__ u32x4_t max_bf16x8(u32x4_t a, u32x4_t b) {
    u32x4_t r;
#pragma unroll
    for (int k = 0; k < 4; ++k) r[k] = pack_bf2(fmaxf(bf_lo(a[k]), bf_lo(b[k])), fmaxf(bf_hi(a[k]), bf_hi(b[k])));
    return r;
}

__global__ void maxpool3x3s2_kernel(const bf16_raw* __restrict__ x, int N, int H, int W, int C, bf16_raw* __restrict__ y) {
    const int Ho = (H + 2 - 3) / 2 + 1, Wo = (W + 2 - 3) / 2 + 1;
    const int cv = C / 8;
    const long long total = (long long)N * Ho * Wo * cv;
    for (long long i = (long long)blockIdx.x * blockDim.x + threadIdx.x; i < total; i += (long long)gridDim.x * blockDim.x) {
        const int c = (int)(i % cv);
        long long t = i / cv;
        const int ox = (int)(t % Wo);
        t /= Wo;
        const int oy = (int)(t % Ho);
        const int n = (int)(t / Ho);
        const unsigned int NEG = 0xff80ff80u;
        u32x4_t m = {NEG, NEG, NEG, NEG};
#pragma unroll
        for (int r = 0; r < 3; ++r) {
            const int iy = 2 * oy - 1 + r;
            if (iy < 0 || iy >= H) continue;
#pragma unroll
            for (int s = 0; s < 3; ++s) {
                const int ix = 2 * ox - 1 + s;
                if (ix < 0 || ix >= W) continue;
                const u32x4_t v = *reinterpret_cast<const u32x4_t*>(x + (((long long)n * H + iy) * W + ix) * C + c * 8);
                m = max_bf16x8(m, v);
            }
        }
        *reinterpret_cast<u32x4_t*>(y + i * 8) = m;
    }
}

__device__ __forceinline__ void up2_taps(int o, int n, int& i0, int& i1, float& w0, float& w1) {
    const int j = o >> 1;
    if (o & 1) { i0 = j; i1 = j + 1 < n ? j + 1 : n - 1; w0 = 0.75f; w1 = 0.25f; }
    else       { i0 = j - 1 >= 0 ? j - 1 : 0; i1 = j; w0 = 0.25f; w1 = 0.75f; }
}

__global__ void upsample2x_add_fwd_kernel(const bf16_raw* __restrict__ top, long long top_ppi, long long top_off,
                                          bf16_raw* __restrict__ lat, long long lat_ppi, long long lat_off,
                                          int N, int H, int W, int C) {
    const int cv = C / 8, H2 = 2 * H, W2 = 2 * W;
    const long long total = (long long)N * H2 * W2 * cv;
    for (long long i = (long long)blockIdx.x * blockDim.x + threadIdx.x; i < total; i += (long long)gridDim.x * blockDim.x) {
        const int c = (int)(i % cv);
        long long t = i / cv;
        const int x = (int)(t % W2);
        t /= W2;
        const int y = (int)(t % H2);
        const int n = (int)(t / H2);
        int y0, y1, x0, x1; float wy0, wy1, wx0, wx1;
        up2_taps(y, H, y0, y1, wy0, wy1);
        up2_taps(x, W, x0, x1, wx0, wx1);
        const bf16_raw* tb = top + ((long long)n * top_ppi + top_off) * C + c * 8;
        const u32x4_t a = *reinterpret_cast<const u32x4_t*>(tb + ((long long)y0 * W + x0) * C);
        const u32x4_t b = *reinterpret_cast<const u32x4_t*>(tb + ((long long)y0 * W + x1) * C);
        const u32x4_t cc = *reinterpret_cast<const u32x4_t*>(tb + ((long long)y1 * W + x0) * C);
        const u32x4_t d = *reinterpret_cast<const u32x4_t*>(tb + ((long long)y1 * W + x1) * C);
        bf16_raw* lp = lat + (((long long)n * lat_ppi + lat_off) + (long long)y * W2 + x) * C + c * 8;
        u32x4_t l = *reinterpret_cast<u32x4_t*>(lp);
        u32x4_t o;
#pragma unroll
        for (int k = 0; k < 4; ++k) {
            const float lo = wy0 * (wx0 * bf_lo(a[k]) + wx1 * bf_lo(b[k])) + wy1 * (wx0 * bf_lo(cc[k]) + wx1 * bf_lo(d[k]));
            const float hi = wy0 * (wx0 * bf_hi(a[k]) + wx1 * bf_hi(b[k])) + wy1 * (wx0 * bf_hi(cc[k]) + wx1 * bf_hi(d[k]));
            o[k] = pack_bf2(bf_lo(l[k]) + lo, bf_hi(l[k]) + hi);
        }
        *reinterpret_cast<u32x4_t*>(lp) = o;
    }
}

__device__ __forceinline__ float up2_bwd_weight(int o, int j, int n) {
    int i0, i1; float w0, w1;
    up2_taps(o, n, i0, i1, w0, w1);
    float w = 0.f;
    if (i0 == j) w += w0;
    if (i1 == j) w += w1;
    return w;
}

__global__ void upsample2x_add_bwd_kernel(const bf16_raw* __restrict__ dlat, long long lat_ppi, long long lat_off,
                                          bf16_raw* __restrict__ dtop, long long top_ppi, long long top_off,
                                          int N, int H, int W, int C, int accumulate) {
    const int cv = C / 8, H2 = 2 * H, W2 = 2 * W;
    const long long total = (long long)N * H * W * cv;
    for (long long i = (long long)blockIdx.x * blockDim.x + threadIdx.x; i < total; i += (long long)gridDim.x * blockDim.x) {
        const int c = (int)(i % cv);
        long long t = i / cv;
        const int x = (int)(t % W);
        t /= W;
        const int y = (int)(t % H);
        const int n = (int)(t / H);
        float acc[8] = {0.f, 0.f, 0.f, 0.f, 0.f, 0.f, 0.f, 0.f};
        const bf16_raw* lb = dlat + ((long long)n * lat_ppi + lat_off) * C + c * 8;
        for (int oy = 2 * y - 1; oy <= 2 * y + 2; ++oy) {
            if (oy < 0 || oy >= H2) continue;
            const float wy = up2_bwd_weight(oy, y, H);
            if (wy == 0.f) continue;
            for (int ox = 2 * x - 1; ox <= 2 * x + 2; ++ox) {
                if (ox < 0 || ox >= W2) continue;
// ... 436 lines not shown
```

basedet_amd/models/engine.py:

```python
import numpy as np
import torch

from .. import ops
from ..ops import Geom

BN_EPS = 1e-5


class ParamArena:

    def __init__(self, device):
        self.device = device
        self.entries = []
        self.total = 0
        self.w = self.g = self.v = None

    def reserve(self, name, shape):
        n = int(np.prod(shape))
        off = self.total
        self.entries.append((name, tuple(shape), off, n))
        self.total += (n + 63) // 64 * 64
        return len(self.entries) - 1

    def allocate(self):
        self.w = torch.zeros(self.total, dtype=torch.float32, device=self.device)
        self.g = torch.zeros(self.total, dtype=torch.float32, device=self.device)
        self.v = torch.zeros(self.total, dtype=torch.float32, device=self.device)

    def view(self, which, idx):
        _, shape, off, n = self.entries[idx]
        return getattr(self, which)[off:off + n].view(shape)


class ConvLayer:

    def __init__(self, name, cin, cout, k, stride, pad, device, bn_prefix=None, has_bias=False, trainable=True,
                 cout_pad=None):
        self.name, self.cin, self.cout_real, self.k, self.stride, self.pad = name, cin, cout, k, stride, pad
        self.cout = cout_pad or cout
        self.bn_prefix, self.has_bias, self.trainable = bn_prefix, has_bias, trainable
        self.device = device
        self.w = self.b = self.gw = self.gb = None
        self.row_scale = None
        self.w_fwd = torch.empty((self.cout, k * k, cin), dtype=torch.bfloat16, device=device)
        self.w_dgrad = torch.empty((cin, k * k, self.cout), dtype=torch.bfloat16, device=device) if trainable else None
        self._desc_cache = {}
        self.gskip = False
        self._gskip_cache = {}
        self._gskip_ws = None
        self._chain = (None, None, False)
        self._chain_cache = {}
        self.fp8 = False
        self.fp8_dgrad = False
        self.fp8_wgrad = False
        self.fp8_1x1 = False
        self.fp8_1x1_dgrad = False
        self.w_q8 = self.w_scale8 = self.w_q8t = self.w_scale8t = None
        self.act_scale = 1.0
        self.grad_scale = 4096.0
        self.amax_slot = None
        self.probe_ctl = None
        self.q8_scratch = None

    def bind(self, arena, params):
        w = torch.from_numpy(params[self.name + ".weight"]).permute(0, 2, 3, 1).contiguous()
        if self.cout != self.cout_real:
            pad = torch.zeros((self.cout - self.cout_real,) + tuple(w.shape[1:]))
            w = torch.cat([w, pad], 0)
        if self.trainable:
            self.w = arena.view("w", self._wi); self.gw = arena.view("g", self._wi)
            self.w.copy_(w)
        else:
            self.w = w.to(self.device)
        if self.bn_prefix:
            g, b = params[self.bn_prefix + ".weight"], params[self.bn_prefix + ".bias"]
            m, v = params[self.bn_prefix + ".running_mean"], params[self.bn_prefix + ".running_var"]
            scale = g / np.sqrt(v + BN_EPS)
            self.row_scale = torch.from_numpy(scale.astype(np.float32)).to(self.device)
            self.b = torch.from_numpy((b - m * scale).astype(np.float32)).to(self.device)
        elif self.has_bias:
            b = torch.from_numpy(params[self.name + ".bias"])
            if self.cout != self.cout_real:
                b = torch.cat([b, torch.zeros(self.cout - self.cout_real)])
            if self.trainable:
                self.b = arena.view("w", self._bi); self.gb = arena.view("g", self._bi)
                self.b.copy_(b)
            else:
                self.b = b.to(self.device)

    def reserve(self, arena):
        if not self.trainable:
            return
        self._wi = arena.reserve(self.name + ".weight", (self.cout, self.k, self.k, self.cin))
        if self.has_bias:
            self._bi = arena.reserve(self.name + ".bias", (self.cout,))

    def export(self, out):
        out[self.name + ".weight"] = self.w[: self.cout_real].permute(0, 3, 1, 2).contiguous().cpu().numpy()
        if self.has_bias and not self.bn_prefix:
            out[self.name + ".bias"] = self.b[: self.cout_real].cpu().numpy().copy()

    def export_grad(self, out):
        out[self.name + ".weight"] = self.gw[: self.cout_real].permute(0, 3, 1, 2).contiguous().cpu()
        if self.gb is not None:
            out[self.name + ".bias"] = self.gb[: self.cout_real].cpu().clone()

    def enable_fp8(self, q8_scratch, act_scale=1.0, dgrad=False, grad_scale=4096.0, wgrad=False):
        assert self.cin % 16 == 0 and self.cout % 8 == 0
        self.fp8, self.q8_scratch, self.act_scale = True, q8_scratch, float(act_scale)
        self.w_q8 = torch.empty((self.cout, self.k * self.k, self.cin), dtype=torch.uint8, device=self.device)
        self.w_scale8 = torch.empty((self.cout,), dtype=torch.float32, device=self.device)
        if wgrad and self.trainable and self.k == 3 and self.stride == 1 and self.cin % 16 == 0 and self.cout % 16 == 0:
            self.fp8_wgrad, self.grad_scale = True, float(grad_scale)
        if dgrad and self.trainable and self.k == 3 and self.stride == 1 and self.cin > 128 and self.cout % 16 == 0:
            self.fp8_dgrad, self.grad_scale = True, float(grad_scale)
            self.w_q8t = torch.empty((self.cin, self.k * self.k, self.cout), dtype=torch.uint8, device=self.device)
            self.w_scale8t = torch.empty((self.cin,), dtype=torch.float32, device=self.device)

    def enable_fp8_1x1(self, act_scale=1.0, dgrad=False, grad_scale=4096.0, expanding=True):
        assert self.k == 1 and self.stride == 1 and self.cin % 32 == 0 and self.cout % 32 == 0
        self.act_scale, self.grad_scale = float(act_scale), float(grad_scale)
        if self.cin % 128 == 0 and (self.cin >= 2 * self.cout or expanding):
            self.fp8_1x1 = True
            self.w_q8 = torch.empty((self.cout, 1, self.cin), dtype=torch.uint8, device=self.device)
            self.w_scale8 = torch.empty((self.cout,), dtype=torch.float32, device=self.device)
        if dgrad and self.trainable and self.cout % 128 == 0 and (self.cout >= 2 * self.cin or expanding):
            self.fp8_1x1_dgrad = True
            self.w_q8t = torch.empty((self.cin, 1, self.cout), dtype=torch.uint8, device=self.device)
            self.w_scale8t = torch.empty((self.cin,), dtype=torch.float32, device=self.device)

    def pack_fp8(self):
        if self.k == 1 and (self.fp8_1x1 or self.fp8_1x1_dgrad):
            if self.fp8_1x1:
                ops.weight_pack_fp8(self.w, self.row_scale, self.cout, 1, self.cin, self.act_scale, self.w_q8, self.w_scale8)
            if self.fp8_1x1_dgrad:
                ops.weight_pack_fp8_t(self.w, self.row_scale, self.cout, 1, self.cin, self.grad_scale, self.w_q8t, self.w_scale8t)
            return
        ops.weight_pack_fp8(self.w, self.row_scale, self.cout, self.k * self.k, self.cin, self.act_scale, self.w_q8, self.w_scale8)
        if self.fp8_dgrad:
            ops.weight_pack_fp8_t(self.w, self.row_scale, self.cout, self.k * self.k, self.cin, self.grad_scale, self.w_q8t, self.w_scale8t)

    def pack(self):
        ops.weight_pack(self.w, self.row_scale, self.w_fwd, self.w_dgrad, self.cout, self.k * self.k, self.cin)
        if self.fp8 or self.fp8_1x1 or self.fp8_1x1_dgrad:
            self.pack_fp8()

    def desc(self, gin: Geom, gout: Geom):
        key = (gin.N, tuple(gin.H), tuple(gin.W), tuple(gin.off), gin.pix_per_img,
               tuple(gout.H), tuple(gout.W), tuple(gout.off), gout.pix_per_img)
        d = self._desc_cache.get(key)
        if d is None:
            d = ops.conv_desc(gin, gout, self.cin, self.cout, self.k, self.k, self.stride, self.pad)
            self._desc_cache[key] = d
        return d

    def bwd_desc(self, gin: Geom, gout: Geom):
        d = self.desc(gin, gout)
        if not self.gskip:
            return d
        h = self._gskip_cache.get(id(d))
        if h is None:
            n = (max(ops.conv2d_dgrad_gskip_bytes(d), 4) + 3) // 4
            if self._gskip_ws is None or self._gskip_ws.numel() < n:
                self._gskip_ws = torch.empty(n, dtype=torch.int32, device=self.device)
                self._gskip_cache.clear()
            h = self._gskip_cache[id(d)] = (ops.gskip_desc(d, self._gskip_ws), d)
        gmap, dxmap, clean = self._chain
        if gmap is None and dxmap is None:
            return h[0]
        key = (id(d), self._gskip_ws.data_ptr(), gmap.data_ptr() if gmap is not None else 0, dxmap.data_ptr() if dxmap is not None else 0, clean)
        c = self._chain_cache.get(key)
        if c is None:
            if len(self._chain_cache) > 64:
                self._chain_cache.clear()
            c = self._chain_cache[key] = (ops.gskip_desc(d, self._gskip_ws, gmap=gmap, dxmap=dxmap, dx_clean=clean), d)
        return c[0]

    def set_chain(self, gmap=None, dxmap=None, dx_clean=False):
        self._chain = (gmap, dxmap, bool(dx_clean) and dxmap is not None) if self.gskip else (None, None, False)

    def forward(self, x, gin, gout, y, add=None, relu=False, bits=None, x8=None, y8=None, q_scale=1.0):
        flags = (ops.EPI_RELU if relu else 0) | (ops.EPI_ADD_BEFORE if add is not None else 0)
        if self.fp8_1x1 and x8 is not None and ops.conv1x1_fp8_ok(self.desc(gin, gout), 0):
            return ops.conv1x1_fp8(self.desc(gin, gout), 0, x8, self.w_q8, self.w_scale8, self.b, y, add=add, bits=bits, y8=y8,
                                   q_scale=q_scale, flags=flags)
        if self.fp8 and bits is None:
            xq = x8 if x8 is not None else ops.quantize_fp8(x, self.act_scale, self.q8_scratch(x.numel())[: x.numel()])
            return ops.conv2d_fwd_fp8(self.desc(gin, gout), xq, self.w_q8, self.w_scale8, self.b, y, add=add, flags=flags, y8=y8,
                                      q_scale=self.act_scale)
        return ops.conv2d_fwd(self.desc(gin, gout), x, self.w_fwd, self.b, y, add=add, flags=flags, bits=bits,
                              y8=y8 if (y8 is not None and ops.dense_1x1_bits_ok(self.desc(gin, gout))) else None, q_scale=q_scale)

    def gnstats_ok(self):
        return (not self.fp8) and self.k == 3 and self.stride == 1 and self.pad == 1 and self.cout == 256 and self.cin % 64 == 0

    def forward_gnstats(self, x, gin, gout, y, part):
        return ops.conv2d_fwd_gnstats(self.desc(gin, gout), x, self.w_fwd, self.b, y, part)

    def dgrad(self, g, gin, gout, dx, first=True, mask=None, add_after=None, maskbits=None, g8=None, dx8=None, q_scale=1.0,
              add_before=None, sparse=False):
        flags, add = 0, None
        if add_after is not None:
            flags |= ops.EPI_ADD_AFTER
            add = add_after
        elif add_before is not None:
            flags |= ops.EPI_ADD_BEFORE
            add = add_before
        elif not first:
            flags |= ops.EPI_ADD_BEFORE
            add = dx
            if sparse and self.stride > 1:
                flags |= ops.EPI_SPARSE
        if mask is not None or maskbits is not None:
            flags |= ops.EPI_MASK
        if maskbits is not None:
            mask = None
        d = self.bwd_desc(gin, gout)
        if self.amax_slot is not None and self.probe_ctl[0] and (self.fp8_1x1_dgrad or self.fp8_dgrad):
            ops.absmax_bf16(g, self.amax_slot)
        if self.fp8_1x1_dgrad and g8 is not None and ops.conv1x1_fp8_ok(d, 1):
            ops.conv1x1_fp8(d, 1, g8, self.w_q8t, self.w_scale8t, None, dx, add=add, mask=mask, maskbits=maskbits, y8=dx8,
                            q_scale=q_scale, flags=flags)
            return dx8 is not None
        if self.fp8_dgrad and maskbits is None:
            gq = g8 if g8 is not None else ops.quantize_bf8(g, self.grad_scale, self.q8_scratch(g.numel())[: g.numel()])
            ops.conv2d_dgrad_fp8(d, gq, self.w_q8t, self.w_scale8t, dx, add=add, mask=mask, flags=flags, dx8=dx8, q_scale=q_scale)
            return dx8 is not None
        if dx8 is not None and not ops.dense_1x1_bits_ok(d):
            dx8 = None
        ops.conv2d_dgrad(d, g, self.w_dgrad, dx, add=add, mask=mask, flags=flags, maskbits=maskbits, dx8=dx8, q_scale=q_scale)
        return dx8 is not None

    def dgrad_writes_twin(self, gin, gout):
        return self.fp8_dgrad or ops.dense_1x1_bits_ok(self.desc(gin, gout))

    def wgrad(self, x, g, gin, gout, ws, colsum_ws=None, x8=None, g8=None, queue=None):
        d = self.bwd_desc(gin, gout)
        if self.fp8_wgrad and x8 is not None and g8 is not None:
            ops.conv2d_wgrad_fp8(d, x8, g8, 1.0 / (self.act_scale * self.grad_scale), self.gw, ws, row_scale=self.row_scale)
            if self.gb is not None:
                ops.colsum_bf16(g, g.shape[0], self.cout, self.gb, colsum_ws)
            return
        if queue is not None:
            queue.wgrad(d, x, g, self.gw, self.gb, ws, row_scale=self.row_scale)
        elif self.gb is not None:
            ops.conv2d_wgrad_bias(d, x, g, self.gw, self.gb, ws, row_scale=self.row_scale)
        else:
            ops.conv2d_wgrad(d, x, g, self.gw, ws, row_scale=self.row_scale)

    def thin_backward_ok(self, gin: Geom):
        return (self.k == 1 and self.stride == 1 and self.pad == 0 and self.cin == 256 and self.cout == 16 and self.trainable
                and self.row_scale is None and self.gb is not None and not (self.fp8 or self.fp8_1x1)
                and sum(h * w for h, w in zip(gin.H, gin.W)) == gin.pix_per_img)

    def thin_forward(self, x, gin: Geom, y):
        ops.conv1x1_thin_fwd(x, self.w, self.b, gin.pixels, self.cin, self.cout, y)

    def thin_backward(self, x, g, gin: Geom, dx, ws):
        ops.conv1x1_thin_bwd(x, g, self.w, gin.pixels, self.cin, self.cout, dx, self.gw, self.gb, self.cout_real, ws)

    def wgrad_ws_bytes(self, gin, gout):
        d = self.bwd_desc(gin, gout)
        n = ops.conv2d_wgrad_bias_workspace_bytes(d) if self.gb is not None else ops.conv2d_wgrad_workspace_bytes(d)
        return max(n, ops.conv2d_wgrad_fp8_workspace_bytes(d)) if self.fp8_wgrad else n


class FusedPredConv(ConvLayer):

    def __init__(self, name, parts, cin, k, stride, pad, device, cout_pad):
        self.parts = parts
        super().__init__(name, cin, sum(c for _, c in parts), k, stride, pad, device, has_bias=True, trainable=True, cout_pad=cout_pad)

    def bind(self, arena, params):
        merged = dict(params)
        merged[self.name + ".weight"] = np.concatenate([params[n + ".weight"] for n, _ in self.parts], 0)
        merged[self.name + ".bias"] = np.concatenate([params[n + ".bias"] for n, _ in self.parts], 0)
        super().bind(arena, merged)

    def export(self, out):
        o = 0
        for n, c in self.parts:
            out[n + ".weight"] = self.w[o:o + c].permute(0, 3, 1, 2).contiguous().cpu().numpy()
            out[n + ".bias"] = self.b[o:o + c].cpu().numpy().copy()
            o += c

    def export_grad(self, out):
        o = 0
        for n, c in self.parts:
            out[n + ".weight"] = self.gw[o:o + c].permute(0, 3, 1, 2).contiguous().cpu()
            out[n + ".bias"] = self.gb[o:o + c].cpu().clone()
            o += c


def cls_ld(K):
    return (int(K) + 7) // 8 * 8


def pad_class_rows(a, A, K):
    ld = cls_ld(K)
    a = np.asarray(a)
    assert a.shape[0] == A * K, (a.shape, A, K)
    if ld == K:
        return a
    out = np.zeros((A, ld) + a.shape[1:], a.dtype)
    out[:, :K] = a.reshape((A, K) + a.shape[1:])
    return out.reshape((A * ld,) + a.shape[1:])


def unpad_class_rows(a, A, K):
    ld = cls_ld(K)
    assert a.shape[0] == A * ld, (a.shape, A, K)
    if ld == K:
        return a
    return a.reshape((A, ld) + tuple(a.shape[1:]))[:, :K].reshape((A * K,) + tuple(a.shape[1:]))


class PaddedClsConv(ConvLayer):

    def __init__(self, name, cin, A, K, k, stride, pad, device):
        self.A, self.K, self.cls_ld = int(A), int(K), cls_ld(K)
        super().__init__(name, cin, self.A * self.K, k, stride, pad, device, has_bias=True, trainable=True, cout_pad=self.A * self.cls_ld)

    def bind(self, arena, params):
        w = pad_class_rows(np.asarray(params[self.name + ".weight"], np.float32), self.A, self.K)
        b = pad_class_rows(np.asarray(params[self.name + ".bias"], np.float32), self.A, self.K)
        self.w = arena.view("w", self._wi); self.gw = arena.view("g", self._wi)
        self.w.copy_(torch.from_numpy(w).permute(0, 2, 3, 1).contiguous())
        self.b = arena.view("w", self._bi); self.gb = arena.view("g", self._bi)
        self.b.copy_(torch.from_numpy(b))

    def export(self, out):
        out[self.name + ".weight"] = unpad_class_rows(self.w, self.A, self.K).permute(0, 3, 1, 2).contiguous().cpu().numpy()
# ... 80 lines not shown
```

basedet_amd/models/free_anchor.py:

```python
import torch

from .. import ops
from ..utils.registry import registers
from .retinanet import RetinaNet


@registers.models.register()
class FreeAnchor(RetinaNet):
    MAX_CLASSES = 128

    @classmethod
    def check_config(cls, cfg):
        super().check_config(cfg)
        if cfg.DATA.NUM_CLASSES > cls.MAX_CLASSES:
            raise ValueError(f"DATA.NUM_CLASSES = {cfg.DATA.NUM_CLASSES} is not supported by FreeAnchor: the bag-loss kernel holds at most "
                             f"{cls.MAX_CLASSES} classes per anchor in its LDS tile")

    def get_losses(self, inputs):
        assert self.training
        pre = self.pre_process(inputs)
        pl = pre["plan"]
        self._cur = pl
        self.network_forward(pl)
        m = self.cfg.MODEL
        gt = pre["gt_boxes"]
        num_gt = pre["img_info"][:, 4].to(torch.int32).contiguous()
        N, Gmax = gt.shape[0], gt.shape[1]
        bucket = m.BUCKET.BUCKET_SIZE
        need = ops.freeanchor_workspace_bytes(N, Gmax, bucket, pl.A_total)
        ws = self._scratch("freeanchor", need)
        ops.freeanchor_loss_fwd_bwd(pl.logits, pl.offsets, self.box_ld, self.num_anchors, pl.anchors, self.num_classes, gt, num_gt,
                                    m.BOX_REG.MEAN, m.BOX_REG.STD, m.BUCKET.BOX_IOU_THRESH, bucket, m.LOSSES.SMOOTH_L1_BETA,
                                    m.LOSSES.REG_LOSS_WEIGHT, m.LOSSES.FOCAL_LOSS_ALPHA, m.LOSSES.FOCAL_LOSS_GAMMA, pl.loss_buf,
                                    pl.d_logits, pl.d_offsets, ws, cls_ld=self.cls_ld if self.cls_ld != self.num_classes else None)
        pos_loss, neg_loss = pl.loss_buf[0], pl.loss_buf[1]
        return {"total_loss": pos_loss + neg_loss, "pos_loss": pos_loss, "neg_loss": neg_loss}
```

basedet_amd/models/retinanet.py:

```python
import torch

from .. import ops
from ..streams import fork, join
from ..utils.registry import registers
from . import params as P
from .engine import PaddedClsConv
from .fpn_base import FPNDetector, _round_up


@registers.models.register()
class RetinaNet(FPNDetector):
    @staticmethod
    def init_params(cfg, seed=0):
        return P.init_retinanet_params(cfg, seed)

    @classmethod
    def check_config(cls, cfg):
        super().check_config(cfg)
        if not cfg.MODEL.HEAD.get("WITH_NORM", True):
            raise ValueError("MODEL.HEAD.WITH_NORM = False is not supported for the RetinaNet family: only True (the default) is implemented")

    def _build_head(self, add, params):
        m = self.cfg.MODEL
        ch = self.fpn_ch
        self.num_anchors = len(m.ANCHOR.SCALES[0]) * len(m.ANCHOR.RATIOS[0])
        nc = m.HEAD.NUM_CONVS
        self.cls_tower = [add(f"head.cls_subnet.{2 * i}", ch, ch, 3, 1, 1, bias=True) for i in range(nc)]
        self.box_tower = [add(f"head.bbox_subnet.{2 * i}", ch, ch, 3, 1, 1, bias=True) for i in range(nc)]
        A, K = self.num_anchors, self.num_classes
        self.cls_score = self.convs["head.cls_score"] = PaddedClsConv("head.cls_score", ch, A, K, 3, 1, 1, self.device)
        self.cls_ld = self.cls_score.cls_ld
        self.box_ld = _round_up(A * 4, 8)
        self.bbox_pred = add("head.bbox_pred", ch, A * 4, 3, 1, 1, bias=True, cout_pad=self.box_ld)
        if bool(m.get("SPARSE_BOX_BWD", True)) and m.get("WEIGHT_DTYPE", "bf16") == "bf16":
            for c in self.box_tower + [self.bbox_pred]:
                c.gskip = True
        self.sparse_chain = bool(m.get("SPARSE_BOX_CHAIN", True))
        self._build_base_anchors()

    def _head_convs(self):
        return self.cls_tower + self.box_tower + [self.cls_score, self.bbox_pred]

    def _plan_head(self, pl):
        ch = self.fpn_ch
        N = pl.N
        C = pl._carve
        bf = torch.bfloat16

        def act(g, c):
            return C.empty((g.pixels, c), bf)

        nc = len(self.cls_tower)
        pl.cls_act = [act(pl.pyr, ch) for _ in range(nc)]
        pl.box_act = [act(pl.pyr, ch) for _ in range(nc)]
        A, K = self.num_anchors, self.num_classes
        pl.logits = act(pl.pyr, A * self.cls_ld)
        pl.offsets = act(pl.pyr, self.box_ld)
        pl.d_logits = C.like(pl.logits)
        pl.d_offsets = C.like(pl.offsets)
        pl.g_tower = [[act(pl.pyr, ch) for _ in range(nc)] for _ in range(2)]
        pl.g_map = None
        if self.sparse_chain and all(c.gskip for c in self.box_tower + [self.bbox_pred]):
            nb = ops.conv2d_gskip_map_bytes(self.box_tower[0].desc(pl.pyr, pl.pyr))
            if nb:
                pl.g_map = [C.empty(((nb + 3) // 4,), torch.int32) for _ in range(nc)]
        pl.chain_epoch = None
        tw = lambda: C.empty((pl.pyr.pixels, ch), torch.uint8)
        pl.cls_act8 = [tw() if c.fp8 else None for c in self.cls_tower]
        pl.box_act8 = [tw() if c.fp8 else None for c in self.box_tower]
        tg = self.fp8_grad_twins
        pl.g_tower8 = [[tw() if (c.fp8_dgrad and tg) else None for c in tower] for tower in (self.cls_tower, self.box_tower)]
        pl.g_P8 = tw() if (tg and all(t[0].fp8_dgrad for t in (self.cls_tower, self.box_tower))) else None
        self._plan_anchors(pl)
        tot = pl.A_total
        pl.labels = C.empty((N, tot), torch.int32)
        pl.match_idx = C.empty((N, tot), torch.int32)
        pl.gt_offsets = C.empty((N, tot, 4), torch.float32)
        pl.num_fg = C.zeros((1,), torch.int32)
        pl.loss_buf = C.zeros((2,), torch.float32)

    def head_forward(self, pl):
        concurrent = bool(self.cfg.MODEL.get("HEAD_TOWERS_CONCURRENT", True)) and self.weight_dtype != "fp8_e4m3"
        side = self.streams.aux() if concurrent else None
        with fork(side):
            t, t8 = pl.P, getattr(pl, "P8", None)
            for c, a, a8 in zip(self.box_tower, pl.box_act, pl.box_act8):
                c.forward(t, pl.pyr, pl.pyr, a, relu=True, x8=t8, y8=a8); t, t8 = a, a8
            self.bbox_pred.forward(t, pl.pyr, pl.pyr, pl.offsets, x8=t8)
        t, t8 = pl.P, getattr(pl, "P8", None)
        for c, a, a8 in zip(self.cls_tower, pl.cls_act, pl.cls_act8):
            c.forward(t, pl.pyr, pl.pyr, a, relu=True, x8=t8, y8=a8); t, t8 = a, a8
        self.cls_score.forward(t, pl.pyr, pl.pyr, pl.logits, x8=t8)
        join(side)

    def get_losses(self, inputs):
        assert self.training
        pre = self.pre_process(inputs)
        pl = pre["plan"]
        self._cur = pl
        m = self.cfg.MODEL
        gt = pre["gt_boxes"]
        num_gt = pre["img_info"][:, 4].to(torch.int32).contiguous()
        N, Gmax = gt.shape[0], gt.shape[1]
        ws = self._scratch("assign", N * Gmax * 4).view(torch.float32)
        thr = m.MATCHER.THRESHOLDS
        side = self.streams.aux() if m.get("ASSIGN_ON_SIDE_STREAM", True) else None
        with fork(side):
            ops.retina_assign_encode(pl.anchors, gt, num_gt, thr[0], thr[1], m.MATCHER.ALLOW_LOW_QUALITY, m.BOX_REG.MEAN,
                                     m.BOX_REG.STD, pl.labels, pl.match_idx, pl.gt_offsets, pl.num_fg, ws)
        self.network_forward(pl)
        join(side)
        pl.loss_buf.zero_()
        rows = N * pl.A_total
        ops.focal_loss_fwd_bwd(pl.logits, pl.labels, rows, self.num_classes, m.LOSSES.FOCAL_LOSS_ALPHA,
                               m.LOSSES.FOCAL_LOSS_GAMMA, pl.num_fg, 1.0, pl.loss_buf[0:1], pl.d_logits,
                               ld=self.cls_ld if self.cls_ld != self.num_classes else None)
        ops.smooth_l1_fwd_bwd(pl.offsets, pl.gt_offsets, pl.labels, pl.pyr.pixels, self.num_anchors, self.box_ld,
                              m.LOSSES.SMOOTH_L1_BETA, pl.num_fg, m.LOSSES.REG_LOSS_WEIGHT, pl.loss_buf[1:2], pl.d_offsets)
        cls_loss, reg_loss = pl.loss_buf[0], pl.loss_buf[1]
        return {"total_loss": cls_loss + reg_loss, "cls_loss": cls_loss, "reg_loss": reg_loss}

    def head_backward(self, pl, ws, cws):
        pyr = pl.pyr
        for ti, (tower, acts, pred, dpred) in enumerate(((self.cls_tower, pl.cls_act, self.cls_score, pl.d_logits),
                                                         (self.box_tower, pl.box_act, self.bbox_pred, pl.d_offsets))):
            gbuf, g8 = pl.g_tower[ti], pl.g_tower8[ti]
            n = len(tower)
            maps = pl.g_map if (ti == 1 and self.sparse_chain and all(c.gskip for c in tower + [pred])) else None
            if ti == 1:
                clean = maps is not None and pl.chain_epoch == self.plan_arena.epoch
                pl.chain_epoch = self.plan_arena.epoch if maps is not None else None
                if maps is not None:
                    pred.set_chain(None, maps[n - 1], clean)
                    for i in range(n):
                        tower[i].set_chain(maps[i], maps[i - 1] if i > 0 else None, clean)
            gs = tower[n - 1].grad_scale
            self._wgrad(pred, acts[-1], dpred, pyr, pyr, ws, cws)
            tw = g8[n - 1] if pred.dgrad_writes_twin(pyr, pyr) else None
            if not pred.dgrad(dpred, pyr, pyr, gbuf[n - 1], mask=acts[-1], dx8=tw, q_scale=gs):
                tw = None
            act8 = pl.cls_act8 if ti == 0 else pl.box_act8
            for i in range(n - 1, -1, -1):
                x = acts[i - 1] if i > 0 else pl.P
                x8 = (act8[i - 1] if i > 0 else pl.P8) if tw is not None else None
                self._wgrad(tower[i], x, gbuf[i], pyr, pyr, ws, cws, x8=x8, g8=tw)
                if i > 0:
                    nxt = g8[i - 1] if tower[i].dgrad_writes_twin(pyr, pyr) else None
                    wrote = tower[i].dgrad(gbuf[i], pyr, pyr, gbuf[i - 1], mask=acts[i - 1], g8=tw, dx8=nxt, q_scale=tower[i - 1].grad_scale)
                    tw = nxt if wrote else None
                else:
                    wrote_p = tower[i].dgrad(gbuf[i], pyr, pyr, pl.g_P, first=(ti == 0), g8=tw,
                                             dx8=pl.g_P8 if tower[i].dgrad_writes_twin(pyr, pyr) else None,
                                             q_scale=self.output[self.fpn_stages[0]].grad_scale)
        for c in self.box_tower + [self.bbox_pred]:
            c.set_chain()
        pl.g_P8_ready = pl.g_P8 is not None and bool(wrote_p)

    def _debug_head(self, pl, out, lvl):
        for i in range(pl.pyr.nlev):
            for k in range(len(self.cls_tower)):
                out[f"cls{k}_{i}"] = lvl(pl.cls_act[k], i)
                out[f"box{k}_{i}"] = lvl(pl.box_act[k], i)
            lg = lvl(pl.logits, i)
            out[f"logits_{i}"] = self.cls_score.real_logits(lg.permute(0, 2, 3, 1)).permute(0, 3, 1, 2).contiguous()
            out[f"offs_{i}"] = lvl(pl.offsets, i, self.num_anchors * 4)

    def inference_batch(self, inputs):
        assert not self.training
        pre = self.pre_process(inputs)
        pl = pre["plan"]
        self.network_forward(pl)
        K, A = self.num_classes, self.num_anchors
        m = self.cfg.MODEL
        return self._detect(pl.N, [h * w * A for h, w in pl.sizes], K, 0, pre["img_info"], logits=pl.logits, anchors=pl.anchors,
                            offsets=pl.offsets, off_ld=self.box_ld, A=A, mean=m.BOX_REG.MEAN, std=m.BOX_REG.STD, cls_ld=self.cls_ld)
```

basedet_amd/ops.py:

```python
import ctypes as C
from dataclasses import dataclass, field
from typing import List, Optional

import torch

from . import _lib
from ._lib import ConvDesc, EPI_ADD_AFTER, EPI_ADD_BEFORE, EPI_MASK, EPI_RELU, EPI_SPARSE, check, f32arr, i32arr, ptr, stream_ptr


@dataclass
class Geom:
    N: int
    H: List[int]
    W: List[int]
    off: List[int] = field(default_factory=list)
    pix_per_img: int = 0

    def __post_init__(self):
        if not self.off:
            o = 0
            self.off = []
            for h, w in zip(self.H, self.W):
                self.off.append(o)
                o += h * w
            if not self.pix_per_img:
                self.pix_per_img = o
        if not self.pix_per_img:
            self.pix_per_img = sum(h * w for h, w in zip(self.H, self.W))

    @property
    def nlev(self):
        return len(self.H)

    @property
    def pixels(self):
        return self.N * self.pix_per_img

    def level(self, i):
        return Geom(self.N, [self.H[i]], [self.W[i]], [self.off[i]], self.pix_per_img)

    def conv_out(self, R, stride, pad):
        H = [(h + 2 * pad - R) // stride + 1 for h in self.H]
        W = [(w + 2 * pad - R) // stride + 1 for w in self.W]
        return Geom(self.N, H, W)


def single(N, H, W):
    return Geom(N, [H], [W])


def conv_desc(gin: Geom, gout: Geom, Cin, Cout, R, S, stride, pad) -> ConvDesc:
    d = ConvDesc()
    d.N, d.Cin, d.Cout, d.R, d.S, d.stride, d.pad, d.nseg = gin.N, Cin, Cout, R, S, stride, pad, gin.nlev
    assert gin.nlev == gout.nlev <= _lib.BD_MAX_SEGS
    for i in range(gin.nlev):
        d.Hi[i], d.Wi[i], d.Ho[i], d.Wo[i] = gin.H[i], gin.W[i], gout.H[i], gout.W[i]
        d.in_off[i], d.out_off[i] = gin.off[i], gout.off[i]
    d.in_pix_per_img, d.out_pix_per_img = gin.pix_per_img, gout.pix_per_img
    return d


def L():
    return _lib.load()


_ROUTE = [0, 0, 0, 0]
_SR_SEED = [0]
_ROUTE_NAMES = {"dense1x1": 0, "patch3x3": 1, "wgrad": 2, "fp8_patch": 3}


def set_route(**kw):
    for k, v in kw.items():
        _ROUTE[_ROUTE_NAMES[k]] = 0 if v is None else int(v) + 1


def reset_route():
    _ROUTE[:] = [0, 0, 0, 0]
    _SR_SEED[0] = 0


def _stamp(d):
    d.route[0], d.route[1], d.route[2], d.route[3] = _ROUTE
    d.sr_seed = _SR_SEED[0]
    return d


def conv2d_fwd(d, x, w_packed, bias, y, add=None, flags=0, bits=None, y8=None, q_scale=1.0):
    if y8 is not None:
        check(L().bd_conv2d_fwd_ex(C.byref(_stamp(d)), ptr(x), ptr(w_packed), ptr(bias), ptr(add), ptr(y), ptr(bits), ptr(y8), float(q_scale), flags,
                                   stream_ptr()), "bd_conv2d_fwd_ex")
        return y
    if bits is not None:
        check(L().bd_conv2d_fwd_bits(C.byref(_stamp(d)), ptr(x), ptr(w_packed), ptr(bias), ptr(add), ptr(y), ptr(bits), flags, stream_ptr()),
              "bd_conv2d_fwd_bits")
        return y
    check(L().bd_conv2d_fwd(C.byref(_stamp(d)), ptr(x), ptr(w_packed), ptr(bias), ptr(add), ptr(y), flags, stream_ptr()), "bd_conv2d_fwd")
    return y


def conv2d_dgrad(d, g, w_packed_t, dx, add=None, mask=None, flags=0, maskbits=None, dx8=None, q_scale=1.0):
    if dx8 is not None:
        check(L().bd_conv2d_dgrad_ex(C.byref(_stamp(d)), ptr(g), ptr(w_packed_t), ptr(add), ptr(mask), ptr(maskbits), ptr(dx), ptr(dx8),
                                     float(q_scale), flags, stream_ptr()), "bd_conv2d_dgrad_ex")
        return dx
    if maskbits is not None:
        check(L().bd_conv2d_dgrad_bits(C.byref(_stamp(d)), ptr(g), ptr(w_packed_t), ptr(add), ptr(maskbits), ptr(dx), flags, stream_ptr()),
              "bd_conv2d_dgrad_bits")
        return dx
    check(L().bd_conv2d_dgrad(C.byref(_stamp(d)), ptr(g), ptr(w_packed_t), ptr(add), ptr(mask), ptr(dx), flags, stream_ptr()), "bd_conv2d_dgrad")
    return dx


def conv2d_dgrad_gskip_bytes(d):
    return int(L().bd_conv2d_dgrad_gskip_bytes(C.byref(d)))


def conv2d_gskip_map_bytes(d, of_dx=False):
    return int(L().bd_conv2d_gskip_map_bytes(C.byref(d), int(bool(of_dx))))


def gskip_map_scan(d, t, gmap, of_dx=False):
    check(L().bd_gskip_map_scan(C.byref(d), int(bool(of_dx)), ptr(t), ptr(gmap), gmap.numel() * gmap.element_size(), stream_ptr()),
          "bd_gskip_map_scan")
    return gmap


def gskip_desc(d, scratch=None, gmap=None, dxmap=None, dx_clean=False):
    h = ConvDesc.from_buffer_copy(d)
    h.gskip = 1
    if scratch is not None:
        h.gskip_ws = scratch.data_ptr()
        h.gskip_ws_bytes = scratch.numel() * scratch.element_size()
    if gmap is not None:
        h.gskip_gmap = gmap.data_ptr()
        h.gskip_gmap_bytes = gmap.numel() * gmap.element_size()
    if dxmap is not None:
        h.gskip_dxmap = dxmap.data_ptr()
        h.gskip_dxmap_bytes = dxmap.numel() * dxmap.element_size()
    h.gskip_dx_clean = int(bool(dx_clean))
    return h


def quantize_fp8(x, scale, q):
    check(L().bd_quantize_fp8(ptr(x), x.numel(), float(scale), ptr(q), stream_ptr()), "bd_quantize_fp8")
    return q


def weight_pack_fp8(w, row_scale, Cout, RS, Cin, act_scale, wq, wscale):
    check(L().bd_weight_pack_fp8(ptr(w), ptr(row_scale), Cout, RS, Cin, float(act_scale), ptr(wq), ptr(wscale), stream_ptr()),
          "bd_weight_pack_fp8")


def conv2d_fwd_fp8(d, xq, wq, wscale, bias, y, add=None, flags=0, y8=None, q_scale=1.0):
    check(L().bd_conv2d_fwd_fp8_ex(C.byref(_stamp(d)), ptr(xq), ptr(wq), ptr(wscale), ptr(bias), ptr(add), ptr(y), ptr(y8), float(q_scale), flags,
                                   stream_ptr()), "bd_conv2d_fwd_fp8")
    return y


def quantize_bf8(x, scale, q):
    check(L().bd_quantize_bf8(ptr(x), x.numel(), float(scale), ptr(q), _SR_SEED[0], stream_ptr()), "bd_quantize_bf8")
    return q


def fp8_set_stochastic_rounding(seed):
    _SR_SEED[0] = int(seed) & 0xFFFFFFFF


def absmax_bf16(x, out):
    check(L().bd_absmax_bf16(ptr(x), x.numel(), ptr(out), stream_ptr()), "bd_absmax_bf16")


def weight_pack_fp8_t(w, row_scale, Cout, RS, Cin, grad_scale, wq_t, wscale_t):
    check(L().bd_weight_pack_fp8_t(ptr(w), ptr(row_scale), Cout, RS, Cin, float(grad_scale), ptr(wq_t), ptr(wscale_t), stream_ptr()),
          "bd_weight_pack_fp8_t")


def conv2d_dgrad_fp8(d, g8, wq_t, wscale_t, dx, add=None, mask=None, flags=0, dx8=None, q_scale=1.0):
    check(L().bd_conv2d_dgrad_fp8(C.byref(_stamp(d)), ptr(g8), ptr(wq_t), ptr(wscale_t), ptr(add), ptr(mask), ptr(dx), ptr(dx8), float(q_scale),
                                  flags, stream_ptr()), "bd_conv2d_dgrad_fp8")
    return dx


def conv1x1_fp8(d, mode, xq, wq, wscale, bias, y, add=None, mask=None, maskbits=None, bits=None, y8=None, q_scale=1.0, flags=0):
    check(L().bd_conv1x1_fp8(C.byref(_stamp(d)), mode, ptr(xq), ptr(wq), ptr(wscale), ptr(bias), ptr(add), ptr(mask), ptr(maskbits), ptr(y),
                             ptr(bits), ptr(y8), float(q_scale), flags, stream_ptr()), "bd_conv1x1_fp8")
    return y


def conv2d_wgrad_fp8_workspace_bytes(d):
    return int(L().bd_conv2d_wgrad_fp8_workspace_bytes(C.byref(_stamp(d))))


def conv2d_wgrad_fp8(d, x8, g8, inv_scale, dw, ws, row_scale=None, accumulate=False):
    check(L().bd_conv2d_wgrad_fp8(C.byref(_stamp(d)), ptr(x8), ptr(g8), float(inv_scale), ptr(row_scale), ptr(dw), int(accumulate), ptr(ws),
                                  ws.numel() * ws.element_size(), stream_ptr()), "bd_conv2d_wgrad_fp8")
    return dw


def conv1x1_fp8_ok(d, mode):
    K, CO = (d.Cin, d.Cout) if mode == 0 else (d.Cout, d.Cin)
    return dense_1x1_bits_ok(d) and K % 128 == 0 and CO % 32 == 0


def fp8_dgrad_ok(d):
    same = all(d.Hi[i] == d.Ho[i] and d.Wi[i] == d.Wo[i] for i in range(d.nseg))
    return d.R == 3 and d.S == 3 and d.stride == 1 and d.pad == 1 and same and d.Cin > 128 and d.Cin % 8 == 0 and d.Cout % 16 == 0


def dense_1x1_bits_ok(d):
    return (d.R == 1 and d.S == 1 and d.stride == 1 and d.pad == 0 and d.nseg == 1 and d.in_off[0] == 0 and d.out_off[0] == 0
            and d.in_pix_per_img == d.Hi[0] * d.Wi[0] and d.out_pix_per_img == d.Ho[0] * d.Wo[0]
            and d.Cin % 32 == 0 and d.Cout % 32 == 0 and d.N * d.in_pix_per_img * max(d.Cin, d.Cout) * 2 < 0x7fffffff)


def conv2d_wgrad_workspace_bytes(d):
    return int(L().bd_conv2d_wgrad_workspace_bytes(C.byref(_stamp(d))))


def conv2d_wgrad(d, x, g, dw, ws, row_scale=None, accumulate=False):
    check(L().bd_conv2d_wgrad(C.byref(_stamp(d)), ptr(x), ptr(g), ptr(row_scale), ptr(dw), int(accumulate), ptr(ws),
                              ws.numel() * ws.element_size(), stream_ptr()), "bd_conv2d_wgrad")
    return dw


def conv2d_wgrad_bias_workspace_bytes(d):
    return int(L().bd_conv2d_wgrad_bias_workspace_bytes(C.byref(_stamp(d))))


def conv2d_wgrad_bias(d, x, g, dw, dbias, ws, row_scale=None, accumulate=False):
    check(L().bd_conv2d_wgrad_bias(C.byref(_stamp(d)), ptr(x), ptr(g), ptr(row_scale), ptr(dw), ptr(dbias), int(accumulate), ptr(ws),
                                   ws.numel() * ws.element_size(), stream_ptr()), "bd_conv2d_wgrad_bias")
    return dw


def fpn_deconv_pack(w, C, w_fwd, w_dgrad):
    check(L().bd_fpn_deconv_pack(ptr(w), C, ptr(w_fwd), ptr(w_dgrad), stream_ptr()), "bd_fpn_deconv_pack")


def fpn_deconv_fwd(x, w_fwd, y, N, Hc, Wc, C, add=None):
    check(L().bd_fpn_deconv_fwd(ptr(x), ptr(w_fwd), ptr(add), ptr(y), N, Hc, Wc, 2 * Hc, 2 * Wc, C, stream_ptr()), "bd_fpn_deconv_fwd")
    return y


def fpn_deconv_dgrad(dy, w_dgrad, dx, N, Hc, Wc, C, add=None):
    check(L().bd_fpn_deconv_dgrad(ptr(dy), ptr(w_dgrad), ptr(add), ptr(dx), N, Hc, Wc, 2 * Hc, 2 * Wc, C, stream_ptr()), "bd_fpn_deconv_dgrad")
    return dx


def fpn_deconv_wgrad_workspace_bytes(N, Hc, Wc, C):
    return int(L().bd_fpn_deconv_wgrad_workspace_bytes(N, Hc, Wc, C))


def fpn_deconv_wgrad(x, dy, dw, ws, N, Hc, Wc, C, accumulate=False):
    check(L().bd_fpn_deconv_wgrad(ptr(x), ptr(dy), ptr(dw), int(accumulate), ptr(ws), ws.numel() * ws.element_size(), N, Hc, Wc,
                                  2 * Hc, 2 * Wc, C, stream_ptr()), "bd_fpn_deconv_wgrad")
    return dw


def stem_conv7x7_fwd(N, H, W, x_halo, w_stem, bias, y):
    check(L().bd_stem_conv7x7_fwd(N, H, W, ptr(x_halo), ptr(w_stem), ptr(bias), ptr(y), stream_ptr()), "bd_stem_conv7x7_fwd")
    return y


def stem_weight_pack(w, row_scale, w_stem):
    check(L().bd_stem_weight_pack(ptr(w), ptr(row_scale), ptr(w_stem), stream_ptr()), "bd_stem_weight_pack")


def weight_pack(w, row_scale, w_fwd, w_dgrad, Cout, RS, Cin):
    check(L().bd_weight_pack(ptr(w), ptr(row_scale), ptr(w_fwd), ptr(w_dgrad), Cout, RS, Cin, stream_ptr()), "bd_weight_pack")


def build_pack_table(entries, device):
    import ctypes as C
    import numpy as np
    from ._lib import PackDesc
    arr = (PackDesc * len(entries))()
    start = 0
    for i, (w, rs, wf, wd, co, r, ci) in enumerate(entries):
        arr[i].w = w.data_ptr()
        arr[i].row_scale = rs.data_ptr() if rs is not None else None
        arr[i].w_fwd = wf.data_ptr() if wf is not None else None
        arr[i].w_dgrad = wd.data_ptr() if wd is not None else None
        arr[i].Cout, arr[i].RS, arr[i].Cin, arr[i].block_start = co, r, ci, start
        start += int(L().bd_weight_pack_blocks(co, r, ci))
    raw = np.frombuffer(bytes(arr), dtype=np.uint8).copy()
    return torch.from_numpy(raw).to(device), len(entries), start


def weight_pack_multi(table):
    t, n, blocks = table
    check(L().bd_weight_pack_multi(ptr(t), n, blocks, stream_ptr()), "bd_weight_pack_multi")

# ... 596 lines not shown
```

include/basedet_hip.h:

```cpp
#ifndef BASEDET_HIP_H
#define BASEDET_HIP_H

#include <stddef.h>
#include <stdint.h>

#ifdef __cplusplus
extern "C" {
#endif

#define BD_OK 0
#define BD_EINVAL (-1)
#define BD_ELAUNCH (-2)
#define BD_EWORKSPACE (-3)

#define BD_MAX_SEGS 8

#define BD_EPI_RELU 1
#define BD_EPI_ADD_BEFORE 2
#define BD_EPI_ADD_AFTER 4
#define BD_EPI_MASK 8
#define BD_EPI_SPARSE 16

typedef void* bd_stream_t;

typedef struct bd_conv_desc {
    int32_t N;
    int32_t Cin, Cout;
    int32_t R, S;
    int32_t stride, pad;
    int32_t nseg;
    int32_t Hi[BD_MAX_SEGS], Wi[BD_MAX_SEGS];
    int32_t Ho[BD_MAX_SEGS], Wo[BD_MAX_SEGS];
    int32_t in_off[BD_MAX_SEGS], out_off[BD_MAX_SEGS];
    int32_t in_pix_per_img, out_pix_per_img;
    int32_t route[4];
    uint32_t sr_seed;
    int32_t gskip;
    void* gskip_ws;
    size_t gskip_ws_bytes;
    void* gskip_gmap;
    size_t gskip_gmap_bytes;
    void* gskip_dxmap;
    size_t gskip_dxmap_bytes;
    int32_t gskip_dx_clean;
} bd_conv_desc;

const char* bd_last_error_string(void);
int bd_version(void);
const char* bd_conv_last_kernel(void);
int bd_probe_mfma_rate(double seconds, double* tflops_out, double* clock_mhz_out, bd_stream_t stream);

int bd_probe_kernel_clock(const char* kernel, int reset, double* clock_mhz_out, double* busy_ms_out);


int bd_conv2d_fwd(const bd_conv_desc* d, const void* x, const void* w_packed, const float* bias,
                  const void* add, void* y, int flags, bd_stream_t stream);

int bd_conv2d_dgrad(const bd_conv_desc* d, const void* g, const void* w_packed_t, const void* add,
                    const void* mask, void* dx, int flags, bd_stream_t stream);
size_t bd_conv2d_dgrad_gskip_bytes(const bd_conv_desc* d);
size_t bd_conv2d_gskip_map_bytes(const bd_conv_desc* d, int of_dx);
int bd_gskip_map_scan(const bd_conv_desc* d, int of_dx, const void* t, void* map, size_t map_bytes, bd_stream_t stream);

int bd_conv2d_fwd_bits(const bd_conv_desc* d, const void* x, const void* w_packed, const float* bias, const void* add, void* y,
                       uint32_t* ybits, int flags, bd_stream_t stream);
int bd_conv2d_dgrad_bits(const bd_conv_desc* d, const void* g, const void* w_packed_t, const void* add, const uint32_t* maskbits,
                         void* dx, int flags, bd_stream_t stream);
int bd_conv2d_fwd_ex(const bd_conv_desc* d, const void* x, const void* w_packed, const float* bias, const void* add, void* y,
                     uint32_t* ybits, void* y8, float q_scale, int flags, bd_stream_t stream);
int bd_conv2d_dgrad_ex(const bd_conv_desc* d, const void* g, const void* w_packed_t, const void* add, const void* mask,
                       const uint32_t* maskbits, void* dx, void* dx8, float q_scale, int flags, bd_stream_t stream);

size_t bd_conv2d_wgrad_workspace_bytes(const bd_conv_desc* d);
int bd_conv2d_wgrad(const bd_conv_desc* d, const void* x, const void* g, const float* row_scale, float* dw,
                    int accumulate, void* ws, size_t ws_bytes, bd_stream_t stream);

size_t bd_conv2d_wgrad_bias_workspace_bytes(const bd_conv_desc* d);
int bd_conv2d_wgrad_bias(const bd_conv_desc* d, const void* x, const void* g, const float* row_scale, float* dw, float* dbias,
                         int accumulate, void* ws, size_t ws_bytes, bd_stream_t stream);

typedef struct bd_wgrad_queue* bd_wgrad_queue_t;
int bd_wgrad_queue_create(bd_wgrad_queue_t* out);
int bd_wgrad_queue_destroy(bd_wgrad_queue_t q);
int bd_wgrad_queue_pending(bd_wgrad_queue_t q);
int bd_conv2d_wgrad_queued(bd_wgrad_queue_t q, const bd_conv_desc* d, const void* x, const void* g, const float* row_scale, float* dw,
                           float* dbias, int accumulate, void* ws, size_t ws_bytes, bd_stream_t stream);
int bd_wgrad_queue_flush(bd_wgrad_queue_t q, bd_stream_t stream);



int bd_stem_conv7x7_fwd(int N, int H, int W, const void* x_halo, const void* w_stem, const float* bias,
                        void* y, bd_stream_t stream);
int bd_stem_pool_fwd(int N, int H, int W, const void* x_halo, const void* w_stem, const float* bias, void* y_pool,
                     bd_stream_t stream);
int bd_stem_weight_pack(const float* w , const float* row_scale, void* w_stem,
                        bd_stream_t stream);

int bd_weight_pack(const float* w, const float* row_scale, void* w_fwd, void* w_dgrad, int Cout, int RS,
                   int Cin, bd_stream_t stream);

typedef struct bd_pack_desc {
    const float* w;
    const float* row_scale;
    void* w_fwd;
    void* w_dgrad;
    int32_t Cout, RS, Cin, block_start;
} bd_pack_desc;
int bd_weight_pack_blocks(int Cout, int RS, int Cin);
int bd_weight_pack_multi(const bd_pack_desc* descs_dev, int n, int total_blocks, bd_stream_t stream);

size_t bd_colsum_workspace_bytes(int C);
int bd_colsum_bf16(const void* g, int N, int64_t pix_per_img, int64_t off, int64_t cnt, int C, float* out,
                   int accumulate, void* ws, size_t ws_bytes, bd_stream_t stream);

int bd_bottleneck_fwd_supported(int N, int H, int W, int Cin, int Cmid, int Cout, int has_downsample);
int bd_bottleneck_fwd(int N, int H, int W, int Cin, int Cmid, int Cout, const void* x, const void* w1, const float* b1, const void* w2,
                      const float* b2, const void* w3, const float* b3, const void* wd, const float* bd, void* y, bd_stream_t stream);


int bd_pad_normalize(const float* in, int N, int H, int W, int Hp, int Wp, const float* mean3,
                     const float* std3, void* out, bd_stream_t stream);
typedef struct bd_h2d* bd_h2d_t;
#define BD_HOST_F64 0
#define BD_HOST_F32 1
#define BD_HOST_U8 2
int bd_h2d_create(bd_h2d_t* out, int device, int threads);
int bd_h2d_threads(bd_h2d_t h);
int bd_h2d_submit(bd_h2d_t h, const void* src_host, int src_dtype, int64_t n, float* dst_dev, int64_t chunk_elems, bd_stream_t stream);
int bd_h2d_destroy(bd_h2d_t h);

int bd_pad_normalize_nchw(const float* in, int N, int H, int W, int Hp, int Wp, const float* mean3,
                          const float* std3, float* out, bd_stream_t stream);

typedef struct bd_image_desc {
    int64_t offset;
    int32_t src_h, src_w, dst_h, dst_w, flip;
    int32_t reserved_[1];
} bd_image_desc;
int bd_resize_pad_normalize(const uint8_t* packed_dev, int64_t packed_bytes, const bd_image_desc* descs_host, int N, int Hp, int Wp,
                            const float* mean3, const float* std3, void* x_halo, bd_stream_t stream);

int bd_maxpool3x3s2_fwd(const void* x, int N, int H, int W, int C, void* y, bd_stream_t stream);

int bd_upsample2x_add_fwd(const void* top, int64_t top_pix_per_img, int64_t top_off, void* lateral,
                          int64_t lat_pix_per_img, int64_t lat_off, int N, int H, int W, int C,
                          bd_stream_t stream);
int bd_upsample2x_add_bwd(const void* dlat, int64_t lat_pix_per_img, int64_t lat_off, void* dtop,
                          int64_t top_pix_per_img, int64_t top_off, int N, int H, int W, int C,
                          int accumulate, bd_stream_t stream);

int bd_fpn_deconv_pack(const float* w, int C, void* w_fwd, void* w_dgrad, bd_stream_t stream);
int bd_fpn_deconv_fwd(const void* x, const void* w_fwd, const void* add, void* y, int N, int Hc, int Wc, int Hf, int Wf, int C,
                      bd_stream_t stream);
int bd_fpn_deconv_dgrad(const void* dy, const void* w_dgrad, const void* add, void* dx, int N, int Hc, int Wc, int Hf, int Wf, int C,
                        bd_stream_t stream);
size_t bd_fpn_deconv_wgrad_workspace_bytes(int N, int Hc, int Wc, int C);
int bd_fpn_deconv_wgrad(const void* x, const void* dy, float* dw, int accumulate, void* ws, size_t ws_bytes, int N, int Hc, int Wc,
                        int Hf, int Wf, int C, bd_stream_t stream);

int bd_relu_bf16(const void* x, void* y, int64_t n, bd_stream_t stream);
int bd_relu_bwd_bf16(const void* g, const void* mask, const void* add, void* y, int64_t n, bd_stream_t stream);
int bd_add_bf16(const void* a, const void* b, void* y, int64_t n, bd_stream_t stream);


int bd_anchors_generate(int H, int W, int stride, float offset, const float* base, int A, float* out,
                        bd_stream_t stream);
int bd_points_generate(int H, int W, int stride, float offset, int A, float* out, bd_stream_t stream);

int bd_box_pairwise(const float* b1, int m, const float* b2, int n, int mode, float* out, bd_stream_t stream);

int bd_box_encode(const float* anchors, const float* gt, int64_t n, const float* mean4_host,
                  const float* std4_host, float* out, bd_stream_t stream);
int bd_box_decode(const float* anchors, const float* deltas, int64_t n, const float* mean4_host,
                  const float* std4_host, float* out, bd_stream_t stream);

int bd_retina_assign_encode(const float* anchors, int A, const float* gt_boxes, const int32_t* num_gt, int N,
                            int Gmax, float thr_lo, float thr_hi, int allow_low_quality,
                            const float* mean4_host, const float* std4_host, int32_t* labels,
                            int32_t* match_idx, float* offsets, int32_t* num_fg, void* ws, size_t ws_bytes,
                            bd_stream_t stream);

int bd_fcos_assign(const float* points, int P, const int32_t* lvl_start_host, const float* soi_host,
                   const int32_t* strides_host, int L, float radius, const float* gt_boxes,
                   const int32_t* num_gt, int N, int Gmax, int32_t* labels, float* offsets, float* ctrness,
                   float* stats, bd_stream_t stream);

size_t bd_atss_assign_workspace_bytes(int N, int P);
int bd_atss_assign(const float* points, int P, const int32_t* lvl_start_host, const int32_t* strides_host, int L, int topk,
                   float anchor_scale, const float* gt_boxes, const int32_t* num_gt, int N, int Gmax, int32_t* labels,
                   float* offsets, float* ctrness, float* stats, void* ws, size_t ws_bytes, bd_stream_t stream);

size_t bd_ota_assign_workspace_bytes(int N, int P);
int bd_ota_assign(const float* points, int P, const int32_t* lvl_start_host, const int32_t* strides_host, int L, const void* logits,
                  int K, const void* pred_ltrb, const float* gt_boxes, const int32_t* num_gt, int N, int Gmax, float alpha,
                  float gamma, float reg_weight, float center_radius, int candidate_k, int32_t* labels, float* targets,
                  float* gt_ious, float* stats, void* ws, size_t ws_bytes, bd_stream_t stream);
int bd_ota_assign_ld(const float* points, int P, const int32_t* lvl_start_host, const int32_t* strides_host, int L, const void* logits,
                     int K, int ld, const void* pred_ltrb, const float* gt_boxes, const int32_t* num_gt, int N, int Gmax, float alpha,
                     float gamma, float reg_weight, float center_radius, int candidate_k, int32_t* labels, float* targets,
                     float* gt_ious, float* stats, void* ws, size_t ws_bytes, bd_stream_t stream);

size_t bd_ota_sinkhorn_workspace_bytes(int N, int P, int Gmax);
int bd_ota_assign_sinkhorn(const float* points, int P, const int32_t* lvl_start_host, const int32_t* strides_host, int L,
                           const void* logits, int K, const void* pred_ltrb, const float* gt_boxes, const int32_t* num_gt, int N,
                           int Gmax, float alpha, float gamma, float reg_weight, float center_radius, int topq, float eps, int iters,
                           int32_t* labels, float* targets, float* gt_ious, float* stats, void* ws, size_t ws_bytes,
                           bd_stream_t stream);
int bd_ota_assign_sinkhorn_ld(const float* points, int P, const int32_t* lvl_start_host, const int32_t* strides_host, int L,
                              const void* logits, int K, int ld, const void* pred_ltrb, const float* gt_boxes, const int32_t* num_gt,
                              int N, int Gmax, float alpha, float gamma, float reg_weight, float center_radius, int topq, float eps,
                              int iters, int32_t* labels, float* targets, float* gt_ious, float* stats, void* ws, size_t ws_bytes,
                              bd_stream_t stream);

size_t bd_freeanchor_workspace_bytes(int N, int Gmax, int bucket, int A);
int bd_freeanchor_loss_fwd_bwd(const void* logits, const void* offsets, int box_ld, int anchors_per_pix, const float* anchors,
// ... 241 lines not shown
```

Before: 694.7 images/sec.

## Build box-tower gradient liveness maps statically from anchor labels on side stream

Adds a kernel that derives the box-branch gradient liveness maps for every tower depth directly from the assigned anchor labels, dilating the foreground mask by one pixel per 3x3 conv. It runs on the side stream during label assignment. The dgrad path can then skip the per-layer fill/scan of dx maps when marked ready. This moves liveness bookkeeping off the backward critical path. It relies on box gradients being exactly zero outside labelled anchors, so FreeAnchor opts out.

```diff
diff --git a/basedet_amd/_lib.py b/basedet_amd/_lib.py
--- a/basedet_amd/_lib.py
+++ b/basedet_amd/_lib.py
@@ -7,7 +7,7 @@
 LIB_PATH = os.environ.get("BASEDET_HIP_LIB") or os.path.join(_HERE, "lib", "libbasedet_hip.so")
 
 BD_MAX_SEGS = 8
-ABI_VERSION = 105
+ABI_VERSION = 106
 EPI_RELU, EPI_ADD_BEFORE, EPI_ADD_AFTER, EPI_MASK, EPI_SPARSE = 1, 2, 4, 8, 16
 
 
@@ -27,6 +27,7 @@
         ("gskip", C.c_int32), ("gskip_ws", C.c_void_p), ("gskip_ws_bytes", C.c_size_t),
         ("gskip_gmap", C.c_void_p), ("gskip_gmap_bytes", C.c_size_t), ("gskip_dxmap", C.c_void_p), ("gskip_dxmap_bytes", C.c_size_t),
         ("gskip_dx_clean", C.c_int32),
+        ("gskip_dx_ready", C.c_int32),
     ]
 
 
@@ -54,6 +55,7 @@
     "bd_conv2d_dgrad_gskip_bytes": (_Z, [_D]),
     "bd_conv2d_gskip_map_bytes": (_Z, [_D, _I]),
     "bd_gskip_map_scan": (_I, [_D, _I, _P, _P, _Z, _P]),
+    "bd_gskip_maps_from_labels": (_I, [_D, _P, _L, _I, _I, C.POINTER(C.c_void_p), C.POINTER(C.c_size_t), _P]),
     "bd_conv2d_fwd_bits": (_I, [_D, _P, _P, _P, _P, _P, _P, _I, _P]),
     "bd_conv2d_fwd_ex": (_I, [_D, _P, _P, _P, _P, _P, _P, _P, _F, _I, _P]),
     "bd_conv2d_dgrad_ex": (_I, [_D, _P, _P, _P, _P, _P, _P, _P, _F, _I, _P]),
diff --git a/basedet_amd/csrc/conv3x3_pp.hip b/basedet_amd/csrc/conv3x3_pp.hip
--- a/basedet_amd/csrc/conv3x3_pp.hip
+++ b/basedet_amd/csrc/conv3x3_pp.hip
@@ -115,7 +115,7 @@
         int zt = p.total_patches;
         const int* plist = nullptr;
         if (p.sp_clean) {
-            const int oc = __builtin_amdgcn_readfirstlane(p.sp_ohdr[0]) & 1;
+            const int oc = (__builtin_amdgcn_readfirstlane(p.sp_ohdr[0]) ^ (p.sp_clean >> 1)) & 1;
             const int pc = __builtin_amdgcn_readfirstlane(p.sp_ohdr[2 + oc]);
             zt = pc < 0 ? 0 : (pc < zt ? pc : zt);
             plist = p.sp_olist + oc * p.sp_stride;
@@ -152,7 +152,7 @@
     int z_first = 0;
     const int* sp_list = p.sp_list;
     if constexpr (SPARSE) {
-        if (p.sp_ohdr && blockIdx.x == 0 && threadIdx.x == 0) p.sp_ohdr[1] = 0;
+        if (p.sp_ohdr && p.sp_clean < 2 && blockIdx.x == 0 && threadIdx.x == 0) p.sp_ohdr[1] = 0;
         const int cur = p.sp_hdr ? __builtin_amdgcn_readfirstlane(p.sp_hdr[0]) & 1 : 0;
         const int* cntp = p.sp_hdr ? p.sp_hdr + 2 + cur : p.sp_count;
         n_live = __builtin_amdgcn_readfirstlane(*cntp);
@@ -730,14 +730,15 @@
             bd_gskip_scan(d, src, PH, PW, mk, stream);
             bd_gskip_compact(d, PH, PW, mk, mk + tot, mk + 2 * tot, mk + 3 * tot, stream);
         }
-        if (d->gskip_dxmap) {
+        const bool ready = d->gskip_dx_ready != 0;
+        if (d->gskip_dxmap && (!ready || d->gskip_dx_clean)) {
             BdGskipMap xm;
             bd_gskip_map_layout(d, 1, &xm);
             p.sp_ohdr = (int*)d->gskip_dxmap; p.sp_olist = p.sp_ohdr + xm.list;
-            p.sp_clean = d->gskip_dx_clean ? 1 : 0;
+            p.sp_clean = d->gskip_dx_clean ? (ready ? 2 : 1) : 0;
         }
         hipLaunchKernelGGL((conv3x3_pp_kernel<1, false, true>), dim3(p.main_grid), dim3(512), LDS_BYTES, stream, p);
-        if (d->gskip_dxmap) bd_gskip_fill(d, 1, dst, p.sp_live, (int*)d->gskip_dxmap, stream);
+        if (d->gskip_dxmap && !ready) bd_gskip_fill(d, 1, dst, p.sp_live, (int*)d->gskip_dxmap, stream);
     } else if (gn_part) {
         BD_ONCE_PER_DEVICE((void)hipFuncSetAttribute(reinterpret_cast<const void*>(&conv3x3_pp_kernel<0, true>), hipFuncAttributeMaxDynamicSharedMemorySize, LDS_BYTES));
         hipLaunchKernelGGL((conv3x3_pp_kernel<0, true>), dim3(p.main_grid), dim3(512), LDS_BYTES, stream, p);
diff --git a/basedet_amd/csrc/conv_igemm.hip b/basedet_amd/csrc/conv_igemm.hip
--- a/basedet_amd/csrc/conv_igemm.hip
+++ b/basedet_amd/csrc/conv_igemm.hip
@@ -562,7 +562,7 @@
         BD_REQUIRE(d->gskip_ws && d->gskip_ws_bytes >= need, "conv2d_dgrad: gskip scratch %zu < required %zu bytes (or NULL)",
                    (size_t)d->gskip_ws_bytes, need);
     }
-    if (d->gskip_gmap || d->gskip_dxmap || d->gskip_dx_clean) {
+    if (d->gskip_gmap || d->gskip_dxmap || d->gskip_dx_clean || d->gskip_dx_ready) {
         BD_REQUIRE(d->gskip && is_3x3s1(d) && g_use_patch3x3 && !maskbits && !dx8 && bd_conv3x3_pp_maps_ok(d, flags, add, dx),
                    "conv2d_dgrad: liveness maps need gskip on a 3x3 / stride 1 / pad 1 descriptor into more than 128 channels with an overwriting "
                    "(or, without gskip_dxmap, in-place accumulating) epilogue on the default route");
@@ -571,6 +571,8 @@
         BD_REQUIRE(!d->gskip_dxmap || d->gskip_dxmap_bytes >= bd_conv2d_gskip_map_bytes(d, 1), "conv2d_dgrad: gskip_dxmap %zu < required %zu bytes",
                    (size_t)d->gskip_dxmap_bytes, bd_conv2d_gskip_map_bytes(d, 1));
         BD_REQUIRE(!d->gskip_dx_clean || d->gskip_dxmap, "conv2d_dgrad: gskip_dx_clean needs gskip_dxmap (the list the promise refers to)");
+        BD_REQUIRE(d->gskip_dx_ready == 0 || (d->gskip_dx_ready == 1 && d->gskip_gmap && d->gskip_dxmap),
+                   "conv2d_dgrad: gskip_dx_ready (0 / 1) needs gskip_gmap and gskip_dxmap (the complete maps of g and dx)");
     }
     if (d->stride == 1) flags &= ~BD_EPI_SPARSE;
     BD_REQUIRE(d->Cout % 8 == 0, "conv2d_dgrad: Cout=%d must be a multiple of 8 (pad the gradient)", d->Cout);
diff --git a/basedet_amd/csrc/gskip.hip b/basedet_amd/csrc/gskip.hip
--- a/basedet_amd/csrc/gskip.hip
+++ b/basedet_amd/csrc/gskip.hip
@@ -79,7 +79,7 @@
 }
 
 template <bool FRESH>
-__device__ __forceinline__ void gs_compact_body(const GsParams& p, int* live, int* list, int* count, int* wsum) {
+__device__ __forceinline__ void gs_compact_body(const GsParams& p, const int* mask, int* live, int* list, int* count, int* wsum) {
     constexpr int KP = 8;
     const int tid = threadIdx.x, wv = tid >> 6, ln = tid & 63;
     int base = 0;
@@ -94,7 +94,7 @@
                 const int s = gs_level(p, rem);
                 const int pwn = p.seg[s].pw, rows = (p.seg[s].H + p.ph - 1) / p.ph;
                 const int local = rem - p.seg[s].patch_start, by = local / pwn, bx = local - by * pwn;
-                const int* m = p.mask + (long long)n * p.patches_per_img + p.seg[s].patch_start;
+                const int* m = mask + (long long)n * p.patches_per_img + p.seg[s].patch_start;
                 const bool up = by > 0, dn = by + 1 < rows, lf = bx > 0, rt = bx + 1 < pwn;
                 int v = gs_mask<FRESH>(m, by * pwn + bx) & GS_ANY;
                 if (up) v |= gs_mask<FRESH>(m, (by - 1) * pwn + bx) & GS_BOT;
@@ -139,7 +139,7 @@
 
 __global__ __launch_bounds__(1024) void gskip_compact_kernel(const GsParams p, int* live, int* list, int* count) {
     __shared__ int wsum[16];
-    gs_compact_body<false>(p, live, list, count, wsum);
+    gs_compact_body<false>(p, p.mask, live, list, count, wsum);
 }
 
 enum { GM_HDR = 8 };
@@ -228,8 +228,112 @@
     __builtin_amdgcn_fence(__ATOMIC_ACQUIRE, "agent");
     const int nxt = (p.map[0] & 1) ^ 1;
     int* live = m8 + p.tot8;
-    gs_compact_body<true>(cp, live, live + p.tot4 * (1 + nxt), p.map + 2 + nxt, wsum);
+    gs_compact_body<true>(cp, cp.mask, live, live + p.tot4 * (1 + nxt), p.map + 2 + nxt, wsum);
     if (tid == 0) { p.map[0] = nxt; p.map[1] = 0; }
+}
+
+enum { GB_ROWS = 8, GB_MAXD = 8, GB_MAXW = 4096, GB_WPR = GB_MAXW / 32, GB_BUF = GB_ROWS + 2 * GB_MAXD };
+
+struct GbSeg { int H, W, off, s4, s8, b0; };
+
+struct GbParams {
+    const int* labels;
+    int* map[GB_MAXD + 1];
+    int A, depth, ppi, nseg, pi4, pi8, tot4, tot8, bpi;
+    GbSeg seg[BD_MAX_SEGS];
+};
+
+__global__ __launch_bounds__(1024) void gskip_labels_kernel(const GbParams p) {
+    __shared__ unsigned bits[2][GB_BUF * GB_WPR];
+    const int tid = threadIdx.x, wv = tid >> 6, ln = tid & 63;
+    const int n = blockIdx.x / p.bpi, rem = blockIdx.x - n * p.bpi;
+    int s = 0;
+#pragma unroll
+    for (int k = 1; k < BD_MAX_SEGS; ++k)
+        if (k < p.nseg && rem >= p.seg[k].b0) s = k;
+    const int H = p.seg[s].H, W = p.seg[s].W;
+    const int band = rem - p.seg[s].b0, y0 = band * GB_ROWS;
+    const int D = p.depth, rows = GB_ROWS + 2 * D;
+    const int c64 = (W + 63) >> 6, wp = 2 * c64;
+    const long long img = (long long)n * p.ppi + p.seg[s].off;
+    for (int it = wv; it < rows * c64; it += 16) {
+        const int r = it / c64, c = it - r * c64;
+        const int y = y0 - D + r, x = c * 64 + ln;
+        bool fg = false;
+        if (y >= 0 && y < H && x < W) {
+            const int* lp = p.labels + (img + (long long)y * W + x) * p.A;
+            for (int a = 0; a < p.A; ++a) fg |= lp[a] > 0;
+        }
+        const unsigned long long m = __ballot(fg);
+        if (ln == 0) {
+            bits[0][r * wp + 2 * c] = (unsigned)m;
+            bits[0][r * wp + 2 * c + 1] = (unsigned)(m >> 32);
+        }
+    }
+    __syncthreads();
+    const int sc = (W + 15) >> 4, r4 = (H + 3) >> 2, c8 = (W + 7) >> 3;
+    int cur = 0;
+    for (int k = 0; k <= D; ++k) {
+        const unsigned* b = bits[cur];
+        int* m4 = p.map[k] + GM_HDR;
+        int* m8 = m4 + p.tot4;
+        for (int t = tid; t < 2 * sc + c8; t += 1024) {
+            if (t < 2 * sc) {
+                const int h = t / sc, sx = t - h * sc, by = 2 * band + h;
+                if (by < r4) {
+                    unsigned sg[4];
+#pragma unroll
+                    for (int py = 0; py < 4; ++py) sg[py] = (b[(D + 4 * h + py) * wp + (sx >> 1)] >> ((sx & 1) * 16)) & 0xffffu;
+                    const unsigned any = sg[0] | sg[1] | sg[2] | sg[3];
+                    int w = 0;
+                    if (any)
+                        w = GS_ANY | (sg[0] ? GS_TOP : 0) | (sg[3] ? GS_BOT : 0) | ((any & 1u) ? GS_LEFT : 0) | ((any >> 15) ? GS_RIGHT : 0) |
+                            ((sg[0] & 1u) ? GS_TL : 0) | ((sg[0] >> 15) ? GS_TR : 0) | ((sg[3] & 1u) ? GS_BL : 0) | ((sg[3] >> 15) ? GS_BR : 0);
+                    m4[n * p.pi4 + p.seg[s].s4 + by * sc + sx] = w;
+                }
+            } else {
+                const int cx = t - 2 * sc;
+                unsigned any = 0;
+#pragma unroll
+                for (int py = 0; py < GB_ROWS; ++py) any |= (b[(D + py) * wp + (cx >> 2)] >> ((cx & 3) * 8)) & 0xffu;
+                m8[n * p.pi8 + p.seg[s].s8 + band * c8 + cx] = any != 0;
+            }
+        }
+        if (k == D) break;
+        unsigned* o = bits[cur ^ 1];
+        for (int i = tid; i < rows * wp; i += 1024) {
+            const int r = i / wp, w = i - r * wp;
+            const int y = y0 - D + r, rest = W - w * 32;
+            unsigned v = 0;
+            if (y >= 0 && y < H && rest > 0) {
+                unsigned lo = 0, mid = 0, hi = 0;
+#pragma unroll
+                for (int dr = -1; dr <= 1; ++dr) {
+                    const int rr = r + dr;
+                    if (rr < 0 || rr >= rows) continue;
+                    const unsigned* q = b + rr * wp;
+                    mid |= q[w];
+                    if (w > 0) lo |= q[w - 1];
+                    if (w + 1 < wp) hi |= q[w + 1];
+                }
+                v = mid | (mid << 1) | (mid >> 1) | (lo >> 31) | (hi << 31);
+                if (rest < 32) v &= (1u << rest) - 1u;
+            }
+            o[i] = v;
+        }
+        __syncthreads();
+        cur ^= 1;
+    }
+}
+
+__global__ __launch_bounds__(1024) void gskip_labels_compact_kernel(const GsParams cp, const GbParams p) {
+    __shared__ int wsum[16];
+    int* map = p.map[blockIdx.x];
+    const int nxt = (map[0] & 1) ^ 1;
+    int* live = map + GM_HDR + p.tot4 + p.tot8;
+    __syncthreads();
+    gs_compact_body<false>(cp, map + GM_HDR, live, live + p.tot4 * (1 + nxt), map + 2 + nxt, wsum);
+    if (threadIdx.x == 0) { map[0] = nxt; map[1] = 0; }
 }
 
 GsParams gs_params(const bd_conv_desc* d, int ph, int pw, int side = 0) {
@@ -314,3 +418,37 @@
     BD_CHECK_LAUNCH("bd_gskip_map_scan");
     return BD_OK;
 }
+
+extern "C" int bd_gskip_maps_from_labels(const bd_conv_desc* d, const int32_t* labels, int64_t label_count, int A, int depth,
+                                         void* const* maps_host, const size_t* map_bytes_host, bd_stream_t stream) {
+    BD_REQUIRE(d && labels && maps_host && map_bytes_host, "gskip_maps_from_labels: null pointer");
+    const size_t need = bd_conv2d_gskip_map_bytes(d, 0);
+    BD_REQUIRE(need > 0, "gskip_maps_from_labels: liveness maps belong to 3x3 / stride 1 / pad 1 descriptors");
+    BD_REQUIRE(A >= 1 && depth >= 0 && depth <= GB_MAXD, "gskip_maps_from_labels: A = %d (>= 1), depth = %d (0 .. %d)", A, depth, (int)GB_MAXD);
+    BD_REQUIRE(label_count == (int64_t)d->N * d->out_pix_per_img * A, "gskip_maps_from_labels: %lld labels, the geometry has %lld pixels x %d anchors",
+               (long long)label_count, (long long)d->N * d->out_pix_per_img, A);
+    const GsParams g4 = gs_params(d, 4, 16, 0), g8 = gs_params(d, 8, 8, 0);
+    GbParams p{};
+    p.labels = labels; p.A = A; p.depth = depth; p.ppi = d->out_pix_per_img; p.nseg = d->nseg;
+    p.pi4 = g4.patches_per_img; p.pi8 = g8.patches_per_img; p.tot4 = g4.total; p.tot8 = g8.total;
+    for (int k = 0; k <= depth; ++k) {
+        BD_REQUIRE(maps_host[k] && map_bytes_host[k] >= need, "gskip_maps_from_labels: map %d: %zu < required %zu bytes (or NULL)", k,
+                   maps_host[k] ? map_bytes_host[k] : (size_t)0, need);
+        for (int j = 0; j < k; ++j) BD_REQUIRE(maps_host[j] != maps_host[k], "gskip_maps_from_labels: maps %d and %d are the same buffer", j, k);
+        p.map[k] = (int*)maps_host[k];
+    }
+    int bands = 0;
+    for (int s = 0; s < d->nseg; ++s) {
+        BD_REQUIRE(d->Wo[s] <= GB_MAXW && d->Ho[s] >= 1 && d->Wo[s] >= 1 && (long long)d->out_off[s] + (long long)d->Ho[s] * d->Wo[s] <= d->out_pix_per_img,
+                   "gskip_maps_from_labels: level %d is %d x %d at offset %d of %d pixels (width <= %d)", s, d->Ho[s], d->Wo[s], d->out_off[s],
+                   d->out_pix_per_img, (int)GB_MAXW);
+        p.seg[s] = GbSeg{d->Ho[s], d->Wo[s], d->out_off[s], g4.seg[s].patch_start, g8.seg[s].patch_start, bands};
+        bands += cdiv(d->Ho[s], GB_ROWS);
+    }
+    p.bpi = bands;
+    BD_REQUIRE((long long)bands * d->N < 0x7fffffffll, "gskip_maps_from_labels: too many row bands");
+    if (g4.total > 0) hipLaunchKernelGGL(gskip_labels_kernel, dim3(bands * d->N), dim3(1024), 0, (hipStream_t)stream, p);
+    hipLaunchKernelGGL(gskip_labels_compact_kernel, dim3(depth + 1), dim3(1024), 0, (hipStream_t)stream, g4, p);
+    BD_CHECK_LAUNCH("bd_gskip_maps_from_labels");
+    return BD_OK;
+}
diff --git a/basedet_amd/csrc/image_ops.hip b/basedet_amd/csrc/image_ops.hip
--- a/basedet_amd/csrc/image_ops.hip
+++ b/basedet_amd/csrc/image_ops.hip
@@ -29,7 +29,7 @@
 static thread_local const char* g_bd_last_kernel = "";
 void bd_note_kernel(const char* name) { g_bd_last_kernel = name; }
 extern "C" const char* bd_conv_last_kernel(void) { return g_bd_last_kernel; }
-extern "C" int bd_version(void) { return 105; }
+extern "C" int bd_version(void) { return 106; }
 
 namespace {
 
diff --git a/basedet_amd/models/engine.py b/basedet_amd/models/engine.py
--- a/basedet_amd/models/engine.py
+++ b/basedet_amd/models/engine.py
@@ -48,7 +48,7 @@
         self.gskip = False
         self._gskip_cache = {}
         self._gskip_ws = None
-        self._chain = (None, None, False)
+        self._chain = (None, None, False, False)
         self._chain_cache = {}
         self.fp8 = False
         self.fp8_dgrad = False
@@ -165,19 +165,20 @@
                 self._gskip_ws = torch.empty(n, dtype=torch.int32, device=self.device)
                 self._gskip_cache.clear()
             h = self._gskip_cache[id(d)] = (ops.gskip_desc(d, self._gskip_ws), d)
-        gmap, dxmap, clean = self._chain
+        gmap, dxmap, clean, ready = self._chain
         if gmap is None and dxmap is None:
             return h[0]
-        key = (id(d), self._gskip_ws.data_ptr(), gmap.data_ptr() if gmap is not None else 0, dxmap.data_ptr() if dxmap is not None else 0, clean)
+        key = (id(d), self._gskip_ws.data_ptr(), gmap.data_ptr() if gmap is not None else 0, dxmap.data_ptr() if dxmap is not None else 0, clean, ready)
         c = self._chain_cache.get(key)
         if c is None:
             if len(self._chain_cache) > 64:
                 self._chain_cache.clear()
-            c = self._chain_cache[key] = (ops.gskip_desc(d, self._gskip_ws, gmap=gmap, dxmap=dxmap, dx_clean=clean), d)
+            c = self._chain_cache[key] = (ops.gskip_desc(d, self._gskip_ws, gmap=gmap, dxmap=dxmap, dx_clean=clean, dx_ready=ready), d)
         return c[0]
 
-    def set_chain(self, gmap=None, dxmap=None, dx_clean=False):
-        self._chain = (gmap, dxmap, bool(dx_clean) and dxmap is not None) if self.gskip else (None, None, False)
+    def set_chain(self, gmap=None, dxmap=None, dx_clean=False, dx_ready=False):
+        on = dxmap is not None
+        self._chain = (gmap, dxmap, bool(dx_clean) and on, bool(dx_ready) and on and gmap is not None) if self.gskip else (None, None, False, False)
 
     def forward(self, x, gin, gout, y, add=None, relu=False, bits=None, x8=None, y8=None, q_scale=1.0):
         flags = (ops.EPI_RELU if relu else 0) | (ops.EPI_ADD_BEFORE if add is not None else 0)
diff --git a/basedet_amd/models/free_anchor.py b/basedet_amd/models/free_anchor.py
--- a/basedet_amd/models/free_anchor.py
+++ b/basedet_amd/models/free_anchor.py
@@ -7,6 +7,7 @@
 
 @registers.models.register()
 class FreeAnchor(RetinaNet):
+    BOX_GRAD_GATED_BY_LABELS = False
     MAX_CLASSES = 128
 
     @classmethod
diff --git a/basedet_amd/models/retinanet.py b/basedet_amd/models/retinanet.py
--- a/basedet_amd/models/retinanet.py
+++ b/basedet_amd/models/retinanet.py
@@ -10,6 +10,8 @@
 
 @registers.models.register()
 class RetinaNet(FPNDetector):
+    BOX_GRAD_GATED_BY_LABELS = True
+
     @staticmethod
     def init_params(cfg, seed=0):
         return P.init_retinanet_params(cfg, seed)
@@ -36,6 +38,8 @@
             for c in self.box_tower + [self.bbox_pred]:
                 c.gskip = True
         self.sparse_chain = bool(m.get("SPARSE_BOX_CHAIN", True))
+        self.sparse_static = (self.sparse_chain and bool(m.get("SPARSE_BOX_STATIC", True)) and self.BOX_GRAD_GATED_BY_LABELS
+                              and all(c.gskip for c in self.box_tower + [self.bbox_pred]))
         self._build_base_anchors()
 
     def _head_convs(self):
@@ -64,6 +68,8 @@
             nb = ops.conv2d_gskip_map_bytes(self.box_tower[0].desc(pl.pyr, pl.pyr))
             if nb:
                 pl.g_map = [C.empty(((nb + 3) // 4,), torch.int32) for _ in range(nc)]
+        pl.g_map_off = C.empty((pl.g_map[0].numel(),), torch.int32) if (self.sparse_static and pl.g_map is not None) else None
+        pl.static_builds = 0
         pl.chain_epoch = None
         tw = lambda: C.empty((pl.pyr.pixels, ch), torch.uint8)
         pl.cls_act8 = [tw() if c.fp8 else None for c in self.cls_tower]
@@ -108,6 +114,7 @@
         with fork(side):
             ops.retina_assign_encode(pl.anchors, gt, num_gt, thr[0], thr[1], m.MATCHER.ALLOW_LOW_QUALITY, m.BOX_REG.MEAN,
                                      m.BOX_REG.STD, pl.labels, pl.match_idx, pl.gt_offsets, pl.num_fg, ws)
+            self._build_static_maps(pl)
         self.network_forward(pl)
         join(side)
         pl.loss_buf.zero_()
@@ -120,6 +127,14 @@
         cls_loss, reg_loss = pl.loss_buf[0], pl.loss_buf[1]
         return {"total_loss": cls_loss + reg_loss, "cls_loss": cls_loss, "reg_loss": reg_loss}
 
+    def _build_static_maps(self, pl):
+        if not self.sparse_static or pl.g_map_off is None:
+            return
+        nc = len(self.box_tower)
+        ops.gskip_maps_from_labels(self.box_tower[0].desc(pl.pyr, pl.pyr), pl.labels, self.num_anchors,
+                                   [pl.g_map_off] + [pl.g_map[nc - k] for k in range(1, nc + 1)])
+        pl.static_builds += 1
+
     def head_backward(self, pl, ws, cws):
         pyr = pl.pyr
         for ti, (tower, acts, pred, dpred) in enumerate(((self.cls_tower, pl.cls_act, self.cls_score, pl.d_logits),
@@ -128,12 +143,14 @@
             n = len(tower)
             maps = pl.g_map if (ti == 1 and self.sparse_chain and all(c.gskip for c in tower + [pred])) else None
             if ti == 1:
-                clean = maps is not None and pl.chain_epoch == self.plan_arena.epoch
+                static = maps is not None and pl.g_map_off is not None and pl.static_builds > 0
+                clean = maps is not None and pl.chain_epoch == self.plan_arena.epoch and (not static or pl.static_builds == 1)
                 pl.chain_epoch = self.plan_arena.epoch if maps is not None else None
+                pl.static_builds = 0
                 if maps is not None:
-                    pred.set_chain(None, maps[n - 1], clean)
+                    pred.set_chain(pl.g_map_off if static else None, maps[n - 1], clean, static)
                     for i in range(n):
-                        tower[i].set_chain(maps[i], maps[i - 1] if i > 0 else None, clean)
+                        tower[i].set_chain(maps[i], maps[i - 1] if i > 0 else None, clean, static)
             gs = tower[n - 1].grad_scale
             self._wgrad(pred, acts[-1], dpred, pyr, pyr, ws, cws)
             tw = g8[n - 1] if pred.dgrad_writes_twin(pyr, pyr) else None
diff --git a/basedet_amd/ops.py b/basedet_amd/ops.py
--- a/basedet_amd/ops.py
+++ b/basedet_amd/ops.py
@@ -125,7 +125,18 @@
     return gmap
 
 
-def gskip_desc(d, scratch=None, gmap=None, dxmap=None, dx_clean=False):
+def gskip_maps_from_labels(d, labels, A, maps):
+    n = len(maps)
+    for m in maps:
+        ptr(m)
+    check(L().bd_gskip_maps_from_labels(C.byref(d), ptr(labels), labels.numel(), int(A), n - 1,
+                                        (C.c_void_p * n)(*[m.data_ptr() for m in maps]),
+                                        (C.c_size_t * n)(*[m.numel() * m.element_size() for m in maps]), stream_ptr()),
+          "bd_gskip_maps_from_labels")
+    return maps
+
+
+def gskip_desc(d, scratch=None, gmap=None, dxmap=None, dx_clean=False, dx_ready=False):
     h = ConvDesc.from_buffer_copy(d)
     h.gskip = 1
     if scratch is not None:
@@ -138,6 +149,7 @@
         h.gskip_dxmap = dxmap.data_ptr()
         h.gskip_dxmap_bytes = dxmap.numel() * dxmap.element_size()
     h.gskip_dx_clean = int(bool(dx_clean))
+    h.gskip_dx_ready = int(bool(dx_ready))
     return h
 
 
diff --git a/include/basedet_hip.h b/include/basedet_hip.h
--- a/include/basedet_hip.h
+++ b/include/basedet_hip.h
@@ -43,6 +43,7 @@
     void* gskip_dxmap;
     size_t gskip_dxmap_bytes;
     int32_t gskip_dx_clean;
+    int32_t gskip_dx_ready;
 } bd_conv_desc;
 
 const char* bd_last_error_string(void);
@@ -61,6 +62,8 @@
 size_t bd_conv2d_dgrad_gskip_bytes(const bd_conv_desc* d);
 size_t bd_conv2d_gskip_map_bytes(const bd_conv_desc* d, int of_dx);
 int bd_gskip_map_scan(const bd_conv_desc* d, int of_dx, const void* t, void* map, size_t map_bytes, bd_stream_t stream);
+int bd_gskip_maps_from_labels(const bd_conv_desc* d, const int32_t* labels, int64_t label_count, int A, int depth, void* const* maps_host,
+                              const size_t* map_bytes_host, bd_stream_t stream);
 
 int bd_conv2d_fwd_bits(const bd_conv_desc* d, const void* x, const void* w_packed, const float* bias, const void* add, void* y,
                        uint32_t* ybits, int flags, bd_stream_t stream);
```

After: 700.4 images/sec, median of 6. No clear change (+0.8%).
